# omegaiota/DiffCloth

Hardware: AMD Instinct MI355X
Metric: fwd+bwd steps/sec (node), 10k-vtx cloth+contact, batch=256 (higher is better)
Workload: dtype f32

## Files before the change

diffcloth_amd/capi.py:

```python
import ctypes as C
import os

import numpy as np

_HERE = os.path.dirname(os.path.abspath(__file__))
LIB_PATH = os.path.join(_HERE, "lib", "libdiffcloth_hip.so")

DC_PRIM_SPHERE, DC_PRIM_CAPSULE, DC_PRIM_PLANE, DC_PRIM_BOWL, DC_PRIM_SPHERE_DISCRETIZED = 0, 1, 2, 3, 4


class DcError(RuntimeError):
    pass


class dc_primitive(C.Structure):
    _fields_ = [("kind", C.c_int), ("group", C.c_int), ("center", C.c_double * 3), ("top_offset", C.c_double * 3),
                ("corner2", C.c_double * 3), ("radius", C.c_double), ("length", C.c_double), ("mu", C.c_double), ("rotates", C.c_int)]


class dc_params(C.Structure):
    _fields_ = [("time_step", C.c_double), ("density", C.c_double), ("k_stretch", C.c_double), ("k_bend", C.c_double),
                ("k_att", C.c_double), ("gravity", C.c_double * 3), ("forward_tol", C.c_double),
                ("backward_tol", C.c_double), ("gravity_enabled", C.c_int), ("contact_enabled", C.c_int),
                ("selfcollision_enabled", C.c_int), ("gradient_clipping", C.c_int),
                ("gradient_clipping_threshold", C.c_double), ("pd_iter_cap", C.c_int), ("adjoint_iter_cap", C.c_int),
                ("cg_rel_tol", C.c_double), ("cg_max_iter", C.c_int), ("stall_window", C.c_int),
                ("adjoint_mode", C.c_int), ("adjoint_rel_tol", C.c_double), ("adjoint_block_precond", C.c_int), ("adjoint_fp32_only", C.c_int),
                ("max_self_contacts", C.c_int), ("forward_deflation", C.c_int)]


class dc_step_stats(C.Structure):
    _fields_ = [("converged", C.c_int), ("pd_iters", C.c_int), ("cg_iters", C.c_int), ("prim_contacts", C.c_int),
                ("self_contacts", C.c_int), ("last_xdiff", C.c_float), ("self_overflow", C.c_int)]


class dc_bwd_stats(C.Structure):
    _fields_ = [("converged", C.c_int), ("adjoint_iters", C.c_int), ("cg_iters", C.c_int), ("clipped", C.c_int), ("used_direct", C.c_int),
                ("last_udiff", C.c_float), ("refine_cycles", C.c_int), ("fp64_iters", C.c_int), ("residual_verified", C.c_int), ("workgroups", C.c_int)]


class dc_record(C.Structure):
    _fields_ = [("x", C.POINTER(C.c_double)), ("v", C.POINTER(C.c_double)), ("f", C.POINTER(C.c_double)), ("r", C.POINTER(C.c_double)),
                ("prim", C.POINTER(C.c_int)), ("normal", C.POINTER(C.c_double)), ("x_fixed", C.POINTER(C.c_double)),
                ("self_count", C.POINTER(C.c_int)), ("self_pairs", C.POINTER(C.c_int)), ("self_layer", C.POINTER(C.c_int)),
                ("self_normal", C.POINTER(C.c_double)), ("self_d", C.POINTER(C.c_double))]


EXPORTED_SYMBOLS = [
    "dc_create", "dc_destroy", "dc_last_error", "dc_version", "dc_set_mesh", "dc_set_attachments", "dc_set_params",
    "dc_set_primitives", "dc_build", "dc_default_params", "dc_set_solver", "dc_set_flags", "dc_get_counts", "dc_get_system_matrix",
    "dc_get_vertex_data", "dc_alloc_batch", "dc_set_state", "dc_get_state", "dc_set_mu", "dc_set_uniform_force", "dc_set_vertex_forces", "dc_set_vertex_force_field", "dc_get_force_gradient",
    "dc_step_forward", "dc_get_record", "dc_get_contacts", "dc_get_self_contacts", "dc_step_backward", "dc_rollout_forward",
    "dc_seed_gradient", "dc_rollout_backward", "dc_get_gradient", "dc_get_param_gradients", "dc_get_stats", "dc_sync", "dc_timer_start",
    "dc_timer_stop", "dc_kernel_times", "dc_get_cluster", "dc_set_gradient", "dc_set_fixed_point_schedule", "dc_set_force_schedule",
    "dc_set_seed_schedule", "dc_clear_schedules", "dc_get_states", "dc_get_dxfixed", "dc_get_layout", "dc_get_packet_layout", "dc_comm_unique_id", "dc_comm_init", "dc_allreduce_sum", "dc_comm_destroy",
    "dc_get_deflation", "dc_set_record", "dc_set_trajectory_start", "dc_keep_force_gradients", "dc_get_force_gradients", "dc_use_stream", "dc_set_state_dev", "dc_get_state_dev", "dc_step_forward_dev", "dc_step_backward_dev",
    "dc_get_self_friction_path", "dc_get_adjoint_matrix", "dc_dense_phase_times",
]

_lib = None
_dp = C.POINTER(C.c_double)
_ip = C.POINTER(C.c_int)


def load_library():
    global _lib
    if _lib is None:
        path = os.environ.get("DC_LIB", LIB_PATH)
        if not os.path.exists(path):
            raise DcError(f"{path} not found: run `python -m diffcloth_amd.build` (hipcc, gfx950)")
        lib = C.CDLL(path)
        lib.dc_last_error.restype = C.c_char_p
        lib.dc_version.restype = C.c_char_p
        _lib = lib
    return _lib


def _d(a):
    return a.ctypes.data_as(_dp) if a is not None else None


def _i(a):
    return a.ctypes.data_as(_ip) if a is not None else None


def _f64(a):
    return None if a is None else np.ascontiguousarray(np.asarray(a, dtype=np.float64))


def _i32(a):
    return np.ascontiguousarray(np.asarray(a, dtype=np.int32))


def _stats_to_dict(arr, fields):
    return {f: np.array([getattr(s, f) for s in arr]) for f in fields}


class Engine:

    def __init__(self, device=0):
        self.lib = load_library()
        h = C.c_void_p()
        rc = self.lib.dc_create(C.c_int(device), C.byref(h))
        if rc != 0:
            raise DcError(f"dc_create failed with code {rc}: no HIP device available (there is no CPU fallback)")
        self.h = h
        self.device = device
        self.params = dc_params()
        self.lib.dc_default_params(C.byref(self.params))
        self.N = self.T = self.E = self.Af = 0
        self.B = 0
        self.ngroups = 1

    def close(self):
        if getattr(self, "h", None):
            self.lib.dc_destroy(self.h)
            self.h = None

    def __del__(self):
        try:
            self.close()
        except Exception:
            pass

    def _chk(self, rc):
        if rc != 0:
            raise DcError(f"code {rc}: {self.lib.dc_last_error(self.h).decode()}")

    def set_mesh(self, verts, tris):
        v = _f64(verts).reshape(-1)
        t = _i32(tris).reshape(-1)
        self._chk(self.lib.dc_set_mesh(self.h, C.c_int(v.size // 3), _d(v), C.c_int(t.size // 3), _i(t)))

    def set_attachments(self, vertices):
        a = _i32(vertices).reshape(-1)
        self._chk(self.lib.dc_set_attachments(self.h, C.c_int(a.size), _i(a)))

    def set_params(self, **kw):
        for k, v in kw.items():
            if k == "gravity":
                for d in range(3):
                    self.params.gravity[d] = float(v[d])
            elif hasattr(self.params, k):
                setattr(self.params, k, v)
            else:
                raise KeyError(k)
        self._chk(self.lib.dc_set_params(self.h, C.byref(self.params)))

    def set_solver(self, forward_tol=None, backward_tol=None, gradient_clipping=None, clip_threshold=None, force_direct_adjoint=None):
        p = self.params
        if forward_tol is not None: p.forward_tol = forward_tol
        if backward_tol is not None: p.backward_tol = backward_tol
        if gradient_clipping is not None: p.gradient_clipping = int(gradient_clipping)
        if clip_threshold is not None: p.gradient_clipping_threshold = clip_threshold
        if force_direct_adjoint is not None: p.adjoint_mode = (2 if p.adjoint_mode == 2 else 1) if force_direct_adjoint else 0
        self._chk(self.lib.dc_set_solver(self.h, C.c_double(p.forward_tol), C.c_double(p.backward_tol), C.c_int(p.gradient_clipping),
                                         C.c_double(p.gradient_clipping_threshold), C.c_int(int(p.adjoint_mode in (1, 2)))))

    def set_primitives(self, prims):
        arr = (dc_primitive * max(len(prims), 1))()
        groups = []
        for k, p in enumerate(prims):
            arr[k].kind = p.get("kind", DC_PRIM_SPHERE)
            arr[k].group = p.get("group", k)
            for d in range(3):
                arr[k].center[d] = float(p["center"][d])
                arr[k].top_offset[d] = float(p.get("top_offset", (0, 0, 0))[d])
                arr[k].corner2[d] = float(p.get("corner2", (0, 0, 0))[d])
            arr[k].radius = float(p["radius"])
            arr[k].length = float(p.get("length", 0.0))
            arr[k].mu = float(p.get("mu", 0.0))
            arr[k].rotates = int(p.get("rotates", 0))
            if arr[k].group not in groups:
                groups.append(arr[k].group)
        self.ngroups = max(len(groups), 1)
        self._chk(self.lib.dc_set_primitives(self.h, C.c_int(len(prims)), arr))

    def build(self):
        self._chk(self.lib.dc_build(self.h))
        c = _i32(np.zeros(6))
        self._chk(self.lib.dc_get_counts(self.h, _i(c)))
        self.N, self.T, self.E, self.Af, self.nnz, self.rows = [int(x) for x in c]
        return self

    def system_matrix(self):
        ptr = _i32(np.zeros(self.N + 1)); col = _i32(np.zeros(self.nnz)); val = _f64(np.zeros(self.nnz))
        self._chk(self.lib.dc_get_system_matrix(self.h, _i(ptr), _i(col), _d(val)))
        return ptr, col, val

    def vertex_data(self):
        m = _f64(np.zeros(self.N)); a = _f64(np.zeros(self.N)); r = _f64(np.zeros(self.N))
        self._chk(self.lib.dc_get_vertex_data(self.h, _d(m), _d(a), _d(r)))
        return m, a, r

    def alloc_batch(self, batch, tape_steps):
        self._chk(self.lib.dc_alloc_batch(self.h, C.c_int(batch), C.c_int(tape_steps)))
        self.B = batch
        self.tape = tape_steps

    def _vec(self, a, per):
        a = _f64(a).reshape(-1)
        if a.size != self.B * per:
            raise ValueError(f"expected {self.B}x{per} values, got {a.size}")
        return a

    def set_state(self, slot, x, v):
        x = self._vec(x, 3 * self.N); v = self._vec(v, 3 * self.N)
        self._chk(self.lib.dc_set_state(self.h, C.c_int(slot), _d(x), _d(v)))
# ... 86 lines not shown
        return dict(count=cnt.value, layers=nl.value, pairs=pairs[:n], layer=layer[:n], normal=nrm[:n])

    def step_backward(self, slot, dL_dxnew, dL_dvnew, dL_dxinit=None, dL_dvinit=None, is_start=False):
        n3 = 3 * self.N
        gx = self._vec(dL_dxnew, n3); gv = self._vec(dL_dvnew, n3)
        ix = None if dL_dxinit is None else self._vec(dL_dxinit, n3)
        iv = None if dL_dvinit is None else self._vec(dL_dvinit, n3)
        dx = np.zeros((self.B, n3)); dv = np.zeros((self.B, n3))
        dxf = np.zeros((self.B, max(3 * self.Af, 1))); dmu = np.zeros((self.B, self.ngroups))
        st = (dc_bwd_stats * self.B)()
        self._chk(self.lib.dc_step_backward(self.h, C.c_int(slot), _d(gx), _d(gv), _d(ix), _d(iv), C.c_int(int(is_start)),
                                            _d(dx), _d(dv), _d(dxf), _d(dmu), st))
        out = dict(dL_dx=dx, dL_dv=dv, dL_dxfixed=dxf[:, :3 * self.Af], dL_dmu=dmu)
        out.update(_stats_to_dict(st, ["converged", "adjoint_iters", "cg_iters", "clipped", "used_direct", "last_udiff", "refine_cycles", "fp64_iters", "residual_verified", "workgroups"]))
        return out

    def _tp(self, t, per):
        dev = getattr(self, "device", None)
        import torch
        if t is None:
            return None, 1
        if t.is_cuda and dev is not None and t.device.index != dev:
            raise ValueError(f"tensor on cuda:{t.device.index}, the engine runs on device {dev}")
        if not t.is_cuda or not t.is_contiguous() or t.dtype not in (torch.float32, torch.float64) or t.numel() != per:
            raise ValueError(f"expected a contiguous CUDA float32 / float64 tensor of {per} elements, got {t.dtype} {tuple(t.shape)} on {t.device}")
        return C.c_void_p(t.data_ptr()), int(t.dtype == torch.float32)

    def use_stream(self, stream=None):
        self._chk(self.lib.dc_use_stream(self.h, C.c_void_p(stream.cuda_stream) if stream is not None else None))

    def set_state_dev(self, slot, x, v):
        px, f = self._tp(x, self.B * 3 * self.N); pv, f2 = self._tp(v, self.B * 3 * self.N)
        assert f == f2, "x and v must have one dtype"
        self._chk(self.lib.dc_set_state_dev(self.h, C.c_int(slot), px, pv, C.c_int(f)))

    def get_state_dev(self, slot, x, v):
        px, f = self._tp(x, self.B * 3 * self.N); pv, f2 = self._tp(v, self.B * 3 * self.N)
        assert f == f2, "x and v must have one dtype"
        self._chk(self.lib.dc_get_state_dev(self.h, C.c_int(slot), px, pv, C.c_int(f)))

    def step_forward_dev(self, slot, fixed_pts=None):
        p, f = self._tp(fixed_pts, self.B * 3 * self.Af)
        self._chk(self.lib.dc_step_forward_dev(self.h, C.c_int(slot), p, C.c_int(f)))

    def step_backward_dev(self, slot, gx, gv, dx, dv, dxfixed=None, dmu=None, ix=None, iv=None, is_start=False):
        n = self.B * 3 * self.N
        pgx, f = self._tp(gx, n); pgv, _ = self._tp(gv, n); pdx, f3_ = self._tp(dx, n); pdv, _ = self._tp(dv, n)
        pix, _ = self._tp(ix, n); piv, _ = self._tp(iv, n)
        pxf, _ = self._tp(dxfixed, self.B * 3 * self.Af); pmu, _ = self._tp(dmu, self.B * self.ngroups)
        for t in (gv, dx, dv, ix, iv, dxfixed, dmu):
            assert t is None or t.dtype == gx.dtype, "all tensors of a call must have one dtype"
        self._chk(self.lib.dc_step_backward_dev(self.h, C.c_int(slot), pgx, pgv, pix, piv, C.c_int(int(is_start)), pdx, pdv, pxf, pmu, C.c_int(f)))

    def rollout_forward(self, slot, nsteps):
        self._chk(self.lib.dc_rollout_forward(self.h, C.c_int(slot), C.c_int(nsteps)))

    def seed_gradient(self, slot, target=None, scale=1.0):
        t = None if target is None else _f64(target).reshape(-1)
        self._chk(self.lib.dc_seed_gradient(self.h, C.c_int(slot), _d(t), C.c_double(scale)))

    def set_trajectory_start(self, start_slot):
        self._chk(self.lib.dc_set_trajectory_start(self.h, C.c_int(start_slot)))

    def rollout_backward(self, slot, nsteps):
        self._chk(self.lib.dc_rollout_backward(self.h, C.c_int(slot), C.c_int(nsteps)))

    def set_gradient(self, dL_dx, dL_dv):
        n3 = 3 * self.N
        self._chk(self.lib.dc_set_gradient(self.h, _d(self._vec(dL_dx, n3)), _d(self._vec(dL_dv, n3))))

    def set_fixed_point_schedule(self, slot0, xf):
        xf = np.ascontiguousarray(np.asarray(xf, dtype=np.float64).reshape(-1, self.B, 3 * self.Af))
        self._chk(self.lib.dc_set_fixed_point_schedule(self.h, C.c_int(slot0), C.c_int(xf.shape[0]), _d(xf)))

    def set_force_schedule(self, slot0, nsteps, fu=None, fv_scale=None):
        fu = None if fu is None else np.ascontiguousarray(np.asarray(fu, dtype=np.float64).reshape(nsteps, self.B, 3))
        fs = None if fv_scale is None else np.ascontiguousarray(np.asarray(fv_scale, dtype=np.float64).reshape(nsteps, self.B))
        self._chk(self.lib.dc_set_force_schedule(self.h, C.c_int(slot0), C.c_int(nsteps), _d(fu), _d(fs)))

    def set_seed_schedule(self, slot0, dL_dx, dL_dv=None):
        gx = np.ascontiguousarray(np.asarray(dL_dx, dtype=np.float64).reshape(-1, self.B, 3 * self.N))
        gv = None if dL_dv is None else np.ascontiguousarray(np.asarray(dL_dv, dtype=np.float64).reshape(gx.shape))
        self._chk(self.lib.dc_set_seed_schedule(self.h, C.c_int(slot0), C.c_int(gx.shape[0]), _d(gx), _d(gv)))

    def clear_schedules(self):
        self._chk(self.lib.dc_clear_schedules(self.h))

    def get_states(self, slot0, nslots):
        x = np.zeros((nslots, self.B, 3 * self.N)); v = np.zeros((nslots, self.B, 3 * self.N))
        self._chk(self.lib.dc_get_states(self.h, C.c_int(slot0), C.c_int(nslots), _d(x), _d(v)))
        return x, v

    def get_dxfixed(self, slot0, nslots):
        out = np.zeros((nslots, self.B, max(3 * self.Af, 1)))
        if self.Af > 0:
            out = np.zeros((nslots, self.B, 3 * self.Af))
            self._chk(self.lib.dc_get_dxfixed(self.h, C.c_int(slot0), C.c_int(nslots), _d(out)))
        return out[:, :, :3 * self.Af]

    def get_gradient(self):
        dx = np.zeros((self.B, 3 * self.N)); dv = np.zeros((self.B, 3 * self.N)); dmu = np.zeros((self.B, self.ngroups))
        self._chk(self.lib.dc_get_gradient(self.h, _d(dx), _d(dv), _d(dmu)))
        return dx, dv, dmu

    def get_mu_gradient(self):
        dmu = np.zeros((self.B, self.ngroups))
        self._chk(self.lib.dc_get_gradient(self.h, None, None, _d(dmu)))
        return dmu

    def get_param_gradients(self, slot):
        out = np.zeros((self.B, 8))
        self._chk(self.lib.dc_get_param_gradients(self.h, C.c_int(slot), _d(out)))
        return dict(dL_dk=out[:, 0:3], dL_ddensity=out[:, 3], sum_dfext=out[:, 4:7])

    def get_stats(self, slot):
        f = (dc_step_stats * self.B)(); b = (dc_bwd_stats * self.B)()
        self._chk(self.lib.dc_get_stats(self.h, C.c_int(slot), f, b))
        return (_stats_to_dict(f, ["converged", "pd_iters", "cg_iters", "prim_contacts", "self_contacts", "last_xdiff", "self_overflow"]),
                _stats_to_dict(b, ["converged", "adjoint_iters", "cg_iters", "clipped", "used_direct", "last_udiff", "refine_cycles", "fp64_iters", "residual_verified", "workgroups"]))

    def sync(self):
        self._chk(self.lib.dc_sync(self.h))

    @staticmethod
    def comm_unique_id():
        lib = load_library()
        buf = C.create_string_buffer(128)
        rc = lib.dc_comm_unique_id(buf)
        if rc != 0:
            raise DcError(f"code {rc}: dc_comm_unique_id failed (RCCL not available?)")
        return buf.raw

    def comm_init(self, nranks, rank, unique_id):
        self._chk(self.lib.dc_comm_init(self.h, C.c_int(nranks), C.c_int(rank), C.c_char_p(unique_id)))

    def allreduce_sum(self, values):
        a = np.ascontiguousarray(np.asarray(values, dtype=np.float64).reshape(-1)).copy()
        self._chk(self.lib.dc_allreduce_sum(self.h, _d(a), C.c_int(a.size)))
        return a

    def comm_destroy(self):
        self._chk(self.lib.dc_comm_destroy(self.h))

    def layout(self):
        c = _i32(np.zeros(6))
        self._chk(self.lib.dc_get_layout(self.h, _i(c)))
        return dict(renumbered=bool(c[0]), bandwidth=int(c[1]), packet_kernel=bool(c[2]), element_windows=bool(c[3]), windows=int(c[4]), dense_inverse=bool(c[5]))

    def packet_byte_offsets(self):
        k = C.c_int()
        self._chk(self.lib.dc_get_packet_layout(self.h, C.byref(k)))
        return bool(k.value)

    def deflation(self):
        k = C.c_int(); pi = C.c_int()
        self._chk(self.lib.dc_get_deflation(self.h, C.byref(k), C.byref(pi)))
        return k.value, pi.value

    def cluster(self):
        k = C.c_int(); nb = C.c_int()
        self._chk(self.lib.dc_get_cluster(self.h, C.byref(k), C.byref(nb)))
        return k.value

    def self_friction_path(self, reset=False):
        out = np.zeros((self.B, 2), dtype=np.int32)
        self._chk(self.lib.dc_get_self_friction_path(self.h, _i(out), C.c_int(int(reset))))
        return out

    def timer_start(self):
        self._chk(self.lib.dc_timer_start(self.h))

    def timer_stop(self):
        ms = C.c_float()
        self._chk(self.lib.dc_timer_stop(self.h, C.byref(ms)))
        return ms.value

    def adjoint_matrix(self, slot, rollout):
        n = 3 * self.N
        K = np.zeros((n, n))
        self._chk(self.lib.dc_get_adjoint_matrix(self.h, C.c_int(slot), C.c_int(rollout), _d(K)))
        return K

    def dense_phase_times(self, reset=False):
        ms = (C.c_float * 3)()
        self._chk(self.lib.dc_dense_phase_times(self.h, ms, C.c_int(int(reset))))
        return tuple(float(v) for v in ms)

    def kernel_times(self, reset=False):
        a = C.c_float(); b = C.c_float(); na = C.c_int(); nb = C.c_int()
        self._chk(self.lib.dc_kernel_times(self.h, C.byref(a), C.byref(na), C.byref(b), C.byref(nb), C.c_int(int(reset))))
        return dict(fwd_ms=a.value, fwd_launches=na.value, bwd_ms=b.value, bwd_launches=nb.value)
```

diffcloth_amd/csrc/dc_device.h:

```cpp
#pragma once
#include <hip/hip_runtime.h>
#include "../../include/diffcloth_hip.h"

namespace dc {

constexpr int kMaxPrims = 8;
constexpr int kMaxLayers = 4088;
constexpr int kMetaStride = 4096;

#if defined(__HIP_DEVICE_COMPILE__) && defined(DC_KERNEL_TU)
#define DC_G __attribute__((address_space(1)))
#define DC_C __attribute__((address_space(4)))
#else
#define DC_G
#define DC_C
#endif

struct DevPrim {
  int kind, group, rotates, pad;
  float cx, cy, cz, radius;
  float tx, ty, tz, length;
  float ux, uy, uz, pad2;
};

struct DevSystem {
  int N, T, E, Af, NC;
  int nprim, ngroups, pad0;
  const int DC_G *tri_v;
  const float4 DC_G *tri_D;
  const float DC_G *tri_w2;
  const int DC_G *bend_v;
  const float4 DC_G *bend_w;
  const float2 DC_G *bend_nw;
  const int DC_G *att_vertex;
  const int DC_G *att_of_vertex;
  const float DC_G *mass;
  const float DC_G *dinv;
  const int DC_G *P_ptr;
  const int DC_G *P_col;
  const float DC_G *P_val;
  const int DC_G *inc_ptr;
  const int DC_G *inc_idx;
  const int2 DC_G *ell;
  const int DC_G *ell_ptr;
  const int DC_G *ell_w;
  const int4 DC_G *pk;
  const int DC_C *pk_ptr;
  const int DC_C *pk_n;
  const float DC_G *sq_dinv;
  int pk_vpt, pk_ok;
  int pk_threads;
  int pk_ofs;
  int adj_coarse;
  const double DC_G *dsph_tri;
  int dsph_ntri;
  int fwd_defl;
  const float DC_G *defl_u;
  const float DC_G *defl_au;
  const float DC_C *defl_g;
  const float DC_G *dense_inv;
  int dense_ld;
  const int DC_G *user_of;
  const int DC_G *dev_of;
  const int4 DC_C *win;
  const int4 DC_G *wtri_rec;
  const float4 DC_G *wtri_D;
  const int4 DC_G *wbend_rec;
  const float4 DC_G *wbend_w;
  const float4 DC_G *wtri_Dlo;
  const float4 DC_G *wbend_lo;
  const int4 DC_G *winc;
  const int DC_C *winc_ptr;
  const int DC_C *winc_n;
  int nwin, win_vcap, win_nrcap, win_ok;
  int win_lds_bytes, pad2;
  const float DC_G *radii;
  const int DC_G *conn_ptr;
  const int DC_G *conn_idx;
  float max_radii;
  int self_cap;
  int self_lds;
  float h, k_att, gx, gy, gz;
  float k_stretch, k_bend, density;
  int contact_enabled, self_enabled, pad1;
  const double DC_G *tri_D64;
  const double DC_G *tri_w2_64;
  const double DC_G *bend_w64;
  const double DC_G *bend_nw64;
  const double DC_G *mass64;
  const float4 DC_G *tri_Dlo;
  const float4 DC_G *bend_lo;
  double h64, k_att64, k_stretch64, k_bend64, density64;
  double g64[3];
  DevPrim prims[kMaxPrims];
  const DevSystem *self_dev;
};

struct DevWork {
  float *g;
  float *vnow;
  float *vbest;
  float *cg_r, *cg_p, *cg_ap, *cg_x;
  float *corner;
  float4 *ap4;
  float *pre_p, *pre_s;
  float *minv;
  double *u64, *r64, *y64, *x64, *k64[6];
  double *c64;
  int *sd_cell, *sd_order;
  float *sd_sx;
  int2 *sd_rawpair;
  float4 *sd_rawn;
  int *sd_tmp;
};

struct SelfRec {
  int2 *pair;
  float4 *nrm;
  float4 *dvec;
  int *meta;
  int *verts;
};

struct FwdArgs {
  const float *x_in, *v_in;
  float *x_out, *v_out;
  float *rec_f, *rec_r, *rec_n;
  int *rec_prim;
  const float *x_fixed;
  const float *mu;
  const float *fu;
  const float *fv;
  const float *fv_scale;
  const float *fv2;
  dc_step_stats *stats;
  SelfRec self;
  float fwd_tol, cg_tol;
  int pd_cap, cg_max, stall_window;
  int self_full;
  int cg_seed;
  int nsteps, inline_detect;
  size_t slot_state, slot_prim, slot_stats;
  size_t slot_self, slot_meta;
  size_t slot_xfix, slot_fu, slot_fvs;
};

struct BwdArgs {
  const float *x_new;
  const float *rec_f, *rec_n;
  const int *rec_prim;
  SelfRec self;
  const float *mu;
  float *gx, *gv;
  const float *ix, *iv;
  float *d_xfixed;
  float *d_mu;
  float *d_param;
  const float *x_fixed;
  const float *x_prev, *v_prev;
  const float *v_new;
  dc_bwd_stats *stats;
  float bwd_tol, cg_tol, clip_thr, rel_tol;
  int mode;
  int it_cap, cg_max, is_start, clip, stall_window;
  int block_pre;
  int fp32_only;
  int dense_y;
  int verify_all;
  int cg_first;
  int warm;
  int ycap, ybase;
  int nsteps, slot;
  int start_at;
  size_t slot_state, slot_prim, slot_self, slot_meta, slot_param, slot_xf, slot_stats;
  size_t slot_ix;
  const double *inj_x, *inj_f, *inj_n, *inj_sn, *inj_sd;
  float *ys;
};

void launch_pd_step(const DevSystem &S, const DevWork &W, const FwdArgs &A, int B, hipStream_t st);
bool pd_step_fusable(const DevSystem &S);
bool launch_pd_step_packet(const DevSystem &S, const DevWork &W, const FwdArgs &A, int B, hipStream_t st);
bool launch_pd_step_resident(const DevSystem &S, const DevWork &W, const FwdArgs &A, int B, hipStream_t st, int variant);
void launch_self_detect(const DevSystem &S, const DevWork &W, const FwdArgs &A, int B, hipStream_t st);
void launch_adjoint_step(const DevSystem &S, const DevWork &W, const BwdArgs &A, int B, hipStream_t st);
void launch_f64i_to_f32p(const double *src, float *dst, int B, int n, const int *user_of, hipStream_t st);
void launch_f32p_to_f64i(const float *src, double *dst, int B, int n, const int *user_of, hipStream_t st);
void launch_f64i_to_f64p(const double *src, double *dst, int B, int n, const int *user_of, hipStream_t st);
void launch_dev_to_planar(const void *src, int is_f32, float *dst, int B, int n, const int *user_of, hipStream_t st);
void launch_planar_to_dev(const float *src, void *dst, int is_f32, int B, int n, const int *user_of, hipStream_t st);
void launch_copy_cast(const float *src, void *dst, int is_f32, long total, hipStream_t st);
void launch_seed_gradient(const float *x, const float *target, float *gx, float *gv, int B, int N, float scale, hipStream_t st);

}
```

diffcloth_amd/csrc/dc_engine.hip:

```cpp
#include <hip/hip_runtime.h>
#include <algorithm>
#include <cmath>
#include <cstdio>
#include <cstring>
#include <string>
#include <vector>
#include "dc_clusterplan.h"
#include "dc_context.h"
#include "dc_env.h"
#include "dc_record.h"
#include "dc_tables.h"
#include "dc_spheremesh.h"
#include "dc_selftmp.h"

using namespace dc;

namespace dc {
hipError_t launch_pd_step_cluster(const DevSystem &S, const DevCluster &CL, const DevWork &W, const FwdArgs &A, int b0, int nb, hipStream_t st);
hipError_t launch_adjoint_step_cluster(const DevSystem &S, const DevCluster &CL, const DevWork &W, const BwdArgs &A, int b0, int nb, hipStream_t st);
}

static_assert(rec::kMetaStride == kMetaStride && rec::kMaxLayers == kMaxLayers, "dc_record.h restates dc_device.h's record sizes");
static_assert(sizeof(rec::Int2) == sizeof(int2) && alignof(rec::Int2) == alignof(int2), "dc_record.h: Int2 is uploaded as int2");
static_assert(sizeof(rec::Float4) == sizeof(float4) && alignof(rec::Float4) == alignof(float4), "dc_record.h: Float4 is uploaded as float4");
// ... 76 lines not shown
  if (rc) return rc;
  launch_f32p_to_f64i(src, stage, c->B, n_per_rollout, per_vertex ? c->d_user_of : nullptr, c->stream);
  HIPCHK(c, hipMemcpyAsync(dst, stage, elems * sizeof(double), hipMemcpyDeviceToHost, c->stream));
  return DC_OK;
}

int check_batch(dc_ctx *c, int slot_lo, int slot_hi) {
  if (!c->built) return fail(c, DC_ERR_STATE, "dc_build has not been called");
  if (c->B <= 0) return fail(c, DC_ERR_STATE, "dc_alloc_batch has not been called");
  if (slot_lo < 0 || slot_hi > c->tape) return fail(c, DC_ERR_INVALID, "tape slot out of range");
  return DC_OK;
}

int check_self_overflow(dc_ctx *c, const dc_step_stats *st, int slot) {
  for (int b = 0; b < c->B; b++)
    if (st[b].self_overflow)
      return fail(c, DC_ERR_CAPACITY, "self-contact list overflow in the step that produced slot " + std::to_string(slot) + ", rollout " +
                  std::to_string(b) + ((st[b].self_overflow & 1) ? ": more pairs than max_self_contacts = " + std::to_string(c->self_cap) : (st[b].self_overflow & 2) ? std::string(": more than 4088 contact layers") : std::string(": inconsistent contact tables (internal error)")) +
                  " (raise dc_params::max_self_contacts and repeat the step)");
  return DC_OK;
}

FwdArgs fwd_args(dc_ctx *c, int slot) {
  const size_t se = slot_elems(c), sp = (size_t) c->B * c->host.N;
  FwdArgs A;
  A.x_in = c->X + se * slot; A.v_in = c->V + se * slot;
  A.x_out = c->X + se * (slot + 1); A.v_out = c->V + se * (slot + 1);
  A.rec_f = c->F + se * (slot + 1); A.rec_r = c->R + se * (slot + 1); A.rec_n = c->NRM + se * (slot + 1);
  A.rec_prim = c->PRIM + sp * (slot + 1);
  A.x_fixed = c->xf_cur; A.mu = c->mu; A.fu = c->fu_set ? c->fu : nullptr; A.fv = c->fv_set ? c->fv : nullptr;
  A.fv2 = c->fv2_set ? c->fv2 : nullptr;
  A.fv_scale = nullptr; A.slot_xfix = 0; A.slot_fu = 0; A.slot_fvs = 0;
  if (c->S.Af > 0 && c->sched_xf[slot + 1]) A.x_fixed = xf_slot(c, slot + 1);
  if (c->sched_fu[slot + 1]) A.fu = c->FU_S + (size_t) c->B * 3 * (slot + 1);
  if (c->sched_fvs[slot + 1] && A.fv) A.fv_scale = c->FVS_S + (size_t) c->B * (slot + 1);
  A.stats = c->fstats + (size_t) c->B * (slot + 1);
  A.self = self_slot(c, slot + 1);
  A.fwd_tol = (float) c->params.forward_tol;
  A.cg_tol = (float) (c->params.cg_rel_tol > 0 ? c->params.cg_rel_tol : 1e-4);
  A.pd_cap = pd_cap(c);
  A.cg_max = c->params.cg_max_iter > 0 ? c->params.cg_max_iter : 500;
  A.stall_window = c->params.stall_window > 0 ? c->params.stall_window : 0x7fffffff;
  static const bool seed_on = env_not_off("DC_CG_SEED", true);
  A.cg_seed = seed_on ? 1 : 0;
  A.self_full = env_on("DC_FWD_SELFFULL", false);
  A.nsteps = 1; A.inline_detect = 0; A.slot_state = se; A.slot_prim = sp; A.slot_stats = (size_t) c->B;
  A.slot_self = (size_t) c->B * c->self_cap; A.slot_meta = (size_t) c->B * kMetaStride;
  return A;
}
enum class Seeds { none, init, schedule };
BwdArgs bwd_args(dc_ctx *c, int slot, bool is_start, Seeds seeds) {
  const size_t se = slot_elems(c), sp = (size_t) c->B * c->host.N;
  BwdArgs A;
  A.x_new = c->X + se * slot; A.rec_f = c->F + se * slot; A.rec_n = c->NRM + se * slot;
  A.rec_prim = c->PRIM + sp * slot; A.mu = c->mu;
  A.self = self_slot(c, slot);
  A.gx = c->GX; A.gv = c->GV;
  A.ix = nullptr; A.iv = nullptr; A.slot_ix = 0;
  if (seeds == Seeds::init) { A.ix = c->IX; A.iv = c->IV; }
  if (seeds == Seeds::schedule && c->SEEDX && c->sched_seed[slot - 1]) { A.ix = seedx_slot(c, slot - 1); A.iv = seedv_slot(c, slot - 1); A.slot_ix = se; }
  A.d_xfixed = dxf_slot(c, slot); A.d_mu = c->DMU;
  A.d_param = dpar_slot(c, slot);
  A.x_fixed = xf_slot(c, slot);
  A.x_prev = c->X + se * (slot - 1); A.v_prev = c->V + se * (slot - 1); A.v_new = c->V + se * slot; A.stats = c->bstats + (size_t) c->B * slot;
  A.bwd_tol = (float) c->params.backward_tol;
  A.cg_tol = (float) (c->params.cg_rel_tol > 0 ? c->params.cg_rel_tol : 1e-4);
  A.clip_thr = (float) c->params.gradient_clipping_threshold;
  A.it_cap = c->params.adjoint_iter_cap > 0 ? c->params.adjoint_iter_cap : 400;
  A.cg_max = c->params.cg_max_iter > 0 ? c->params.cg_max_iter : 500;
  A.is_start = is_start; A.clip = c->params.gradient_clipping;
  A.start_at = c->start_slot + 1;
  A.mode = c->params.adjoint_mode;
  A.rel_tol = (float) (c->params.adjoint_rel_tol > 0 ? c->params.adjoint_rel_tol : 1e-6);
  A.stall_window = c->params.stall_window > 0 ? c->params.stall_window : 0x7fffffff;
  A.block_pre = env_not_off("DC_BLOCK_PRE", c->params.adjoint_block_precond != 0);
  A.fp32_only = env_on("DC_ADJ_FP32", c->params.adjoint_fp32_only != 0);
  A.dense_y = env_on("DC_ADJ_DENSEY", false);
  A.verify_all = env_on("DC_ADJ_VERIFY", false);
  A.warm = env_on("DC_ADJ_WARM", false);
  A.cg_first = env_on("DC_ADJ_CG", true);
  A.ycap = 0; A.ybase = 0;
  A.nsteps = 1; A.slot = slot;
  const bool inj = c->inj_slot == slot && c->INJ_X;
  A.inj_x = inj ? c->INJ_X : nullptr; A.inj_f = inj ? c->INJ_F : nullptr; A.inj_n = inj ? c->INJ_N : nullptr;
  A.inj_sn = inj ? c->INJ_SN : nullptr; A.inj_sd = inj ? c->INJ_SD : nullptr;
  A.ys = (c->keep_y && c->YS) ? c->YS + se * slot : nullptr;
  A.slot_state = se; A.slot_prim = sp; A.slot_self = (size_t) c->B * c->self_cap; A.slot_meta = (size_t) c->B * kMetaStride;
  A.slot_param = (size_t) c->B * 8; A.slot_xf = xf_elems(c); A.slot_stats = (size_t) c->B;
  return A;
}


void free_cluster(dc_ctx *c) {
  for (void *p : c->cl.allocs) (void) hipFree(p);
  c->cl = ClusterSet();
}

int upload_cluster(dc_ctx *c, const ClusterPlan &P) {
  ClusterSet &cl = c->cl;
  DevCluster &D = cl.D;
  std::memset(&D, 0, sizeof(D));
  D.K = P.K; D.R = P.R; D.HB = P.HB; D.wpp = P.wpp; D.nb = P.nb; D.xch_stride = P.xch_stride; D.pk_vpt = P.pk_vpt;
  D.spin_limit = P.spin_limit; D.redundant_self = P.redundant_self; D.test_drop = P.test_drop; D.test_skew = P.test_skew;
  const HostWindows &HW = P.win;
  const HostPackets &HP = P.pk;
  D.nwin = HW.nwin; D.win_vcap = HW.vcap; D.win_nrcap = HW.nrcap; D.win_lds_bytes = (int) HW.lds_bytes;
  const struct { const void *src; size_t count; void *dst; } tables[] = {
    {HW.win.data(), HW.win.size(), &D.win}, {HW.tri_rec.data(), HW.tri_rec.size(), &D.wtri_rec}, {HW.tri_D.data(), HW.tri_D.size(), &D.wtri_D},
    {HW.bend_rec.data(), HW.bend_rec.size(), &D.wbend_rec}, {HW.bend_w.data(), HW.bend_w.size(), &D.wbend_w},
    {HW.tri_Dlo.data(), HW.tri_Dlo.size(), &D.wtri_Dlo}, {HW.bend_lo.data(), HW.bend_lo.size(), &D.wbend_lo},
    {HW.inc.data(), HW.inc.size(), &D.winc}, {HW.inc_ptr.data(), HW.inc_ptr.size(), &D.winc_ptr}, {HW.inc_n.data(), HW.inc_n.size(), &D.winc_n},
    {HP.pk.data(), HP.pk.size(), &D.pk}, {HP.pk_ptr.data(), HP.pk_ptr.size(), &D.pk_ptr}, {HP.pk_n.data(), HP.pk_n.size(), &D.pk_n},
    {HP.sq_dinv.data(), HP.sq_dinv.size(), &D.sq_dinv}};
  static_assert(sizeof(int) == 4 && sizeof(float) == 4, "4-byte table elements");
  int rc;
  for (const auto &t : tables) {
    int *p = nullptr;
    if ((rc = dev_alloc(c, cl.allocs, &p, t.count))) return rc;
    if (t.count) HIPCHK(c, hipMemcpy(p, t.src, t.count * 4, hipMemcpyHostToDevice));
    std::memcpy(t.dst, &p, sizeof(p));
  }
  if ((rc = dev_alloc(c, cl.allocs, &D.xch, P.xch_bytes / sizeof(v4i)))) return rc;
  if ((rc = dev_alloc(c, cl.allocs, &D.err, 4))) return rc;
  if ((rc = dev_alloc(c, cl.allocs, &D.self_path, 2 * (size_t) c->B))) return rc;
  DevCluster *dD = nullptr;
  if ((rc = dev_alloc(c, cl.allocs, &dD, 1))) return rc;
  D.self_dev = dD;
  HIPCHK(c, hipMemcpy(dD, &D, sizeof(DevCluster), hipMemcpyHostToDevice));
  cl.K = P.K; cl.nb = P.nb; cl.xch_bytes = P.xch_bytes;
  cl.ok = true;
  return DC_OK;
}

static int deflation_want(const dc_params &p) {
  if (env_set("DC_DEFLATION")) return env_int("DC_DEFLATION", 0) > 0 ? 16 : 0;
  return p.forward_deflation > 0 ? 16 : p.forward_deflation;
}
static bool build_deflation_cached(dc_ctx *c, const HostSystem &H, int want, int rows_padded, HostDeflation **out) {
  uint64_t h = 1469598103934665603ull;
  auto mix = [&](const void *q, size_t n) { const unsigned char *b = (const unsigned char *) q; for (size_t i = 0; i < n; i++) { h ^= b[i]; h *= 1099511628211ull; } };
  mix(&H.N, sizeof(int)); mix(&want, sizeof(int)); mix(&rows_padded, sizeof(int));
  mix(H.P_ptr.data(), H.P_ptr.size() * sizeof(H.P_ptr[0])); mix(H.P_col.data(), H.P_col.size() * sizeof(H.P_col[0]));
  mix(H.P_val.data(), H.P_val.size() * sizeof(H.P_val[0])); mix(H.mass.data(), H.mass.size() * sizeof(H.mass[0]));
  if (!c->defl_cache_valid || c->defl_key != h) {
    c->defl_cache_built = c->defl_cache.build(H, want, rows_padded);
    c->defl_key = h; c->defl_cache_valid = true;
  }
  *out = &c->defl_cache;
  return c->defl_cache_built;
}

static void set_decisions(DevSystem &S, const HostTables &plan) {
  S.win_ok = plan.win_ok; S.nwin = plan.nwin; S.pk_ok = plan.pk_ok; S.pk_vpt = plan.pk_vpt; S.pk_threads = plan.pk_threads;
  S.pk_ofs = plan.pk_ofs;
  S.fwd_defl = plan.fwd_defl; S.adj_coarse = plan.adj_coarse; S.dense_ld = plan.dense_ld;
  S.max_radii = plan.max_radii; S.self_cap = plan.self_cap; S.self_lds = plan.self_lds;
}

int choose_cluster(dc_ctx *c) {
  free_cluster(c);
  ClusterSwitches sw;
  sw.forced = env_int("DC_CLUSTER", -1);
  sw.redundant_self = env_on("DC_SELF_REDUNDANT", true);
  sw.spin_ms = env_int("DC_TEST_SPIN_MS", 0);
  sw.test_drop = env_on("DC_TEST_DROP_PART", false);
  sw.test_skew = env_int("DC_TEST_SKEW_PART", -1);
  ClusterPlan plan;
  plan.build(c->host, c->bandwidth, c->B, c->cus, c->host_only, c->S.pk_ok != 0, c->S.win_ok != 0, c->S.dense_inv != nullptr, sw);
  return plan.ok ? upload_cluster(c, plan) : DC_OK;
}

int cluster_check(dc_ctx *c) {
  if (!c->cl.ok) return DC_OK;
  unsigned e[4] = {0, 0, 0, 0};
  HIPCHK(c, hipMemcpy(e, c->cl.D.err, sizeof(e), hipMemcpyDeviceToHost));
  if (e[0]) HIPCHK(c, hipMemset(c->cl.D.err, 0, 16));
  if (e[0]) return fail(c, DC_ERR_HIP, "split kernels: an inter-workgroup exchange timed out (waiting for sequence " + std::to_string(e[1]) + ", saw tag " +
                        std::to_string(e[2]) + ", site " + std::to_string(e[3] & 255u) + ", part " + std::to_string((e[3] >> 8) & 15u) + ", granule " +
                        std::to_string(e[3] >> 12) + "; set DC_CLUSTER=1 to run one workgroup per rollout)");
  return DC_OK;
}

bool use_cluster_fwd(const dc_ctx *c) { return c->cl.ok; }
bool use_cluster_bwd(const dc_ctx *c) { return c->cl.ok && c->params.adjoint_mode == 1; }

int check_dense_mode(dc_ctx *c, int mode, int N, const char *who) {
  if (mode == 2 && N > kDenseMaxN)
    return fail(c, DC_ERR_INVALID, std::string(who) + ": adjoint_mode 2 (dense direct adjoint solve) is limited to meshes of at most " +
                std::to_string(kDenseMaxN) + " vertices; this mesh has " + std::to_string(N));
  return DC_OK;
}

int dense_ensure(dc_ctx *c) {
  if (c->dense.K) return DC_OK;
  const int N = c->host.N, ld = dense_adj_ld(N), cap = std::max(c->self_cap, 1);
  const size_t per = (size_t) ld * ld * sizeof(double) + (size_t) ld * sizeof(int) + sizeof(int) + (size_t) 9 * N * sizeof(double) +
                     (size_t) 9 * cap * sizeof(double);
  const size_t budget = (size_t) 8 << 30;
  int nb = (int) std::max<size_t>(1, std::min<size_t>((size_t) c->B, budget / per));
  const int chunk = env_int("DC_DENSE_CHUNK", 0);
  if (chunk > 0) nb = std::min(nb, chunk);
  int rc;
  DenseAdjWork &D = c->dense;
  D.ld = ld;
  if ((rc = dev_alloc(c, c->batch_allocs, &D.K, (size_t) nb * ld * ld))) return rc;
  if ((rc = dev_alloc(c, c->batch_allocs, &D.piv, (size_t) nb * ld))) return rc;
  if ((rc = dev_alloc(c, c->batch_allocs, &D.flag, (size_t) nb))) return rc;
  if ((rc = dev_alloc(c, c->batch_allocs, &D.pm, (size_t) nb * 9 * N))) return rc;
  if ((rc = dev_alloc(c, c->batch_allocs, &D.sg, (size_t) nb * 9 * cap))) return rc;
  c->dense_nb = nb;
  c->dense_timing = env_on("DC_DENSE_TIMES", false);
  if (c->dense_timing)
    for (auto &e : c->ev_d) if (!e) HIPCHK(c, hipEventCreate(&e));
  return DC_OK;
}

int enqueue_dense_adjoint(dc_ctx *c, const BwdArgs &A) {
  if (A.nsteps != 1) return fail(c, DC_ERR_INVALID, "adjoint_mode 2 runs one backward step per launch");
  int rc;
  if ((rc = dense_ensure(c))) return rc;
  const DenseAdjWork &D = c->dense;
  const int n = 3 * c->host.N;
  static const int one = 1;
  const int forced = env_int("DC_DENSE_FLAG", -1);
  for (int b0 = 0; b0 < c->B; b0 += c->dense_nb) {
    const int nb = std::min(c->dense_nb, c->B - b0);
    if (c->dense_timing) HIPCHK(c, hipEventRecord(c->ev_d[0], c->stream));
    HIPCHK(c, hipMemsetAsync(D.flag, 0, sizeof(int) * nb, c->stream));
    if (forced >= b0 && forced < b0 + nb) HIPCHK(c, hipMemcpyAsync(D.flag + (forced - b0), &one, sizeof(int), hipMemcpyHostToDevice, c->stream));
    launch_dense_assemble(c->S, A, c->W.x64, D, b0, nb, c->stream);
    if (c->dense_timing) HIPCHK(c, hipEventRecord(c->ev_d[1], c->stream));
    c->dense_launches += 2 + launch_dense_factor(D, n, nb, c->stream);
    if (c->dense_timing) HIPCHK(c, hipEventRecord(c->ev_d[2], c->stream));
    launch_dense_adjoint_step(c->S, c->W, A, D, b0, nb, c->stream);
    c->dense_launches += 1;
    HIPCHK(c, hipGetLastError());
    if (c->dense_timing) {
      HIPCHK(c, hipEventRecord(c->ev_d[3], c->stream));
      HIPCHK(c, hipEventSynchronize(c->ev_d[3]));
      for (int k = 0; k < 3; k++) {
        float ms = 0;
        HIPCHK(c, hipEventElapsedTime(&ms, c->ev_d[k], c->ev_d[k + 1]));
        c->dense_ms[k] += ms;
      }
    }
  }
  return DC_OK;
}

int enqueue_pd_step(dc_ctx *c, const FwdArgs &A) {
  {
    const long first = (long) ((A.x_out - c->X) / (long) slot_elems(c));
    if (c->inj_slot >= first && c->inj_slot < first + A.nsteps) c->inj_slot = -1;
  }
  if (!use_cluster_fwd(c)) { launch_pd_step(c->S, c->W, A, c->B, c->stream); HIPCHK(c, hipGetLastError()); return DC_OK; }
  for (int b0 = 0; b0 < c->B; b0 += c->cl.nb) {
    HIPCHK(c, hipMemsetAsync(c->cl.D.xch, 0, c->cl.xch_bytes, c->stream));
    HIPCHK(c, launch_pd_step_cluster(c->S, c->cl.D, c->W, A, b0, std::min(c->cl.nb, c->B - b0), c->stream));
  }
  return DC_OK;
}
int enqueue_adjoint_step(dc_ctx *c, const BwdArgs &A) {
  if (c->params.adjoint_mode == 2) return enqueue_dense_adjoint(c, A);
  if (!use_cluster_bwd(c)) { launch_adjoint_step(c->S, c->W, A, c->B, c->stream); HIPCHK(c, hipGetLastError()); return DC_OK; }
  for (int b0 = 0; b0 < c->B; b0 += c->cl.nb) {
    HIPCHK(c, hipMemsetAsync(c->cl.D.xch, 0, c->cl.xch_bytes, c->stream));
    HIPCHK(c, launch_adjoint_step_cluster(c->S, c->cl.D, c->W, A, b0, std::min(c->cl.nb, c->B - b0), c->stream));
  }
  return DC_OK;
}

bool fuse_steps_enabled() {
  static const bool on = env_not_off("DC_FUSE_STEPS", true);
  return on;
}

int enqueue_forward_steps(dc_ctx *c, int slot, int nsteps, bool carry_targets, int *launches) {
  const bool self_on = c->S.contact_enabled && c->S.self_enabled, has_xf = c->S.Af > 0;
  const bool fused = fuse_steps_enabled() && nsteps > 1 && (use_cluster_fwd(c) || pd_step_fusable(c->S));
  const size_t xf_bytes = sizeof(float) * xf_elems(c);
  int rc;
  FwdArgs FA = fwd_args(c, slot);
  if (fused) {
    int nxf = 0, nfu = 0, nfvs = 0;
    for (int k = 1; k <= nsteps; k++) { nxf += c->sched_xf[slot + k]; nfu += c->sched_fu[slot + k]; nfvs += c->sched_fvs[slot + k]; }
    if ((nxf % nsteps) || (nfu % nsteps) || (nfvs % nsteps))
      return fail(c, DC_ERR_INVALID, "dc_rollout_forward: a fixed-point / force schedule covers only part of the steps " + std::to_string(slot) + " .. " + std::to_string(slot + nsteps));
    if (nxf) FA.slot_xfix = xf_elems(c);
    if (nfu) FA.slot_fu = (size_t) c->B * 3;
    if (nfvs && FA.fv_scale) FA.slot_fvs = (size_t) c->B;
    FA.nsteps = nsteps; FA.inline_detect = self_on ? 1 : 0;
  }
  for (int k = 0; k < nsteps; k++) {
    if (has_xf && !c->sched_xf[slot + k + 1]) HIPCHK(c, hipMemcpyAsync(xf_slot(c, slot + k + 1), c->xf_cur, xf_bytes, hipMemcpyDeviceToDevice, c->stream));
    if (fused) continue;
    if (k) FA = fwd_args(c, slot + k);
    if (self_on) launch_self_detect(c->S, c->W, FA, c->B, c->stream);
    if ((rc = enqueue_pd_step(c, FA))) return rc;
  }
  if (fused && (rc = enqueue_pd_step(c, FA))) return rc;
  if (carry_targets && has_xf && c->sched_xf[slot + nsteps])
    HIPCHK(c, hipMemcpyAsync(c->xf_cur, xf_slot(c, slot + nsteps), xf_bytes, hipMemcpyDeviceToDevice, c->stream));
  if (launches) *launches = fused ? 1 : nsteps;
  return DC_OK;
}

int enqueue_backward_steps(dc_ctx *c, int slot, int nsteps, Seeds seeds, const bool *is_start, int *launches) {
// ... 42 lines not shown

extern "C" {

const char *dc_version(void) { return "diffcloth_hip 0.1 (gfx950)"; }

void dc_default_params(dc_params *p) {
  std::memset(p, 0, sizeof(*p));
  p->time_step = 1.0 / 90; p->density = 0.1; p->k_stretch = 100; p->k_bend = 0.01; p->k_att = 10000;
  p->gravity[0] = 0; p->gravity[1] = -9.8; p->gravity[2] = 0;
  p->forward_tol = 1e-7; p->backward_tol = 5e-5;
  p->gravity_enabled = 1; p->contact_enabled = 1; p->selfcollision_enabled = 0;
  p->gradient_clipping = 1; p->gradient_clipping_threshold = 16.0;
  p->pd_iter_cap = -1; p->adjoint_iter_cap = 400; p->cg_rel_tol = 1e-4; p->cg_max_iter = 500; p->stall_window = 0;
  p->adjoint_mode = 0; p->adjoint_rel_tol = 1e-6; p->adjoint_block_precond = 1; p->adjoint_fp32_only = 0;
  p->max_self_contacts = 0;
  p->forward_deflation = -1;
}

int dc_create(int device_id, dc_ctx **out) {
  if (!out) return DC_ERR_INVALID;
  *out = nullptr;
  if (device_id == -1) {
    dc_ctx *c = new dc_ctx();
    c->device = -1; c->host_only = true;
    dc_default_params(&c->params);
    std::memset(&c->S, 0, sizeof(c->S));
    std::memset(&c->W, 0, sizeof(c->W));
    *out = c;
    return DC_OK;
  }
  int count = 0;
  if (hipGetDeviceCount(&count) != hipSuccess || count <= 0) return DC_ERR_HIP;
  if (device_id < 0 || device_id >= count) return DC_ERR_INVALID;
  dc_ctx *c = new dc_ctx();
  c->device = device_id;
  dc_default_params(&c->params);
  std::memset(&c->S, 0, sizeof(c->S));
  std::memset(&c->W, 0, sizeof(c->W));
  if (hipSetDevice(device_id) != hipSuccess || hipStreamCreate(&c->stream) != hipSuccess) { delete c; return DC_ERR_HIP; }
  c->own_stream = c->stream;
  if (hipDeviceGetAttribute(&c->cus, hipDeviceAttributeMultiprocessorCount, device_id) != hipSuccess || c->cus <= 0) c->cus = 256;
  if (hipEventCreate(&c->ev_a) != hipSuccess || hipEventCreate(&c->ev_b) != hipSuccess || hipEventCreate(&c->ev_t0) != hipSuccess ||
      hipEventCreate(&c->ev_t1) != hipSuccess) { delete c; return DC_ERR_HIP; }
  *out = c;
  return DC_OK;
}

int dc_destroy(dc_ctx *c) {
  if (!c) return DC_OK;
  if (c->host_only) { delete c; return DC_OK; }
  (void) hipSetDevice(c->device);
  (void) hipStreamSynchronize(c->stream);
  (void) dc_comm_destroy(c);
  free_cluster(c);
  free_pool(c->table_allocs);
  free_pool(c->batch_allocs);
  (void) hipEventDestroy(c->ev_a); (void) hipEventDestroy(c->ev_b);
  (void) hipEventDestroy(c->ev_t0); (void) hipEventDestroy(c->ev_t1);
  for (hipEvent_t e : c->ev_d) if (e) (void) hipEventDestroy(e);
  (void) hipStreamDestroy(c->own_stream);
  delete c;
  return DC_OK;
}

const char *dc_last_error(const dc_ctx *c) { return c ? c->err.c_str() : "null context"; }

int dc_set_mesh(dc_ctx *c, int n, const double *pos, int t, const int *tris) {
  if (!c) return DC_ERR_INVALID;
  c->built = false;
  c->user_of.clear(); c->dev_of.clear();
  if (!c->host.set_mesh(n, pos, t, tris)) { c->mesh_set = false; return fail(c, DC_ERR_TOPOLOGY, c->host.error); }
  const bool env = env_set("DC_RENUMBER");
  const bool want = env_on("DC_RENUMBER", 2 * mesh_bandwidth(t, tris) > 511);
  if (want) {
    std::vector<int> order = rcm_order(n, t, tris);
    std::vector<int> inv(n);
    for (int k = 0; k < n; k++) inv[order[k]] = k;
    std::vector<int> tri2(3 * (size_t) t);
    for (size_t k = 0; k < tri2.size(); k++) tri2[k] = inv[tris[k]];
    if (2 * mesh_bandwidth(t, tri2.data()) < 2 * mesh_bandwidth(t, tris) || env) {
      std::vector<double> pos2(3 * (size_t) n);
      for (int k = 0; k < n; k++) for (int d = 0; d < 3; d++) pos2[3 * (size_t) k + d] = pos[3 * (size_t) order[k] + d];
      if (!c->host.set_mesh(n, pos2.data(), t, tri2.data())) { c->mesh_set = false; return fail(c, DC_ERR_TOPOLOGY, c->host.error); }
      c->user_of = order; c->dev_of = inv;
    }
  }
  c->mesh_set = true;
  return DC_OK;
}

int dc_set_attachments(dc_ctx *c, int count, const int *vertex) {
  if (!c || count < 0 || (count > 0 && !vertex)) return fail(c, DC_ERR_INVALID, "dc_set_attachments: bad arguments");
  c->att_user.assign(vertex, vertex + count);
  c->built = false;
  return DC_OK;
}

int dc_set_params(dc_ctx *c, const dc_params *p) {
  if (!c || !p) return DC_ERR_INVALID;
  if (!(p->time_step > 0) || !(p->density > 0)) return fail(c, DC_ERR_INVALID, "dc_set_params: time_step and density must be > 0");
  if (c->mesh_set) { const int rc = check_dense_mode(c, p->adjoint_mode, c->host.N, "dc_set_params"); if (rc) return rc; }
  c->params = *p;
  c->built = false;
  return DC_OK;
}

int dc_set_primitives(dc_ctx *c, int count, const dc_primitive *prims) {
  if (!c || count < 0 || count > kMaxPrims) return fail(c, DC_ERR_INVALID, "dc_set_primitives: at most 8 flattened primitives");
  if (count > 0 && !prims) return fail(c, DC_ERR_INVALID, "dc_set_primitives: null primitive array");
  int discretised = 0;
  for (int k = 0; k < count; k++) {
    if (prims[k].kind < DC_PRIM_SPHERE || prims[k].kind > DC_PRIM_SPHERE_DISCRETIZED) return fail(c, DC_ERR_INVALID, "dc_set_primitives: unknown primitive kind");
    if (prims[k].kind == DC_PRIM_SPHERE_DISCRETIZED) {
      discretised++;
      if (!(prims[k].radius > 0) || prims[k].length < 0 || prims[k].length > 512) return fail(c, DC_ERR_INVALID, "dc_set_primitives: discretised sphere needs radius > 0 and a resolution (length) of 0 or 3 ... 512");
    }
  }
  if (discretised > 1) return fail(c, DC_ERR_INVALID, "dc_set_primitives: at most one discretised sphere per context");
  c->prims.assign(prims, prims + count);
  std::vector<int> seen;
  c->group_of_prim.assign(count, 0);
  for (int k = 0; k < count; k++) {
    int g = -1;
    for (size_t s = 0; s < seen.size(); s++) if (seen[s] == prims[k].group) g = (int) s;
    if (g < 0) { g = (int) seen.size(); seen.push_back(prims[k].group); }
    c->group_of_prim[k] = g;
  }
  c->ngroups = (int) seen.size();
  c->built = false;
  return DC_OK;
}

int dc_build(dc_ctx *c) {
  if (!c) return DC_ERR_INVALID;
  if (!c->mesh_set) return fail(c, DC_ERR_STATE, "dc_build: dc_set_mesh has not been called");
  { const int rc = check_dense_mode(c, c->params.adjoint_mode, c->host.N, "dc_build"); if (rc) return rc; }
  c->inj_slot = -1;
  const dc_params &p = c->params;
  HostSystem &H = c->host;
  H.att_vertex = c->att_user;
  for (int &a : H.att_vertex) {
    if (a < 0 || a >= H.N) return fail(c, DC_ERR_INVALID, "dc_build: attachment vertex out of range");
    if (!c->dev_of.empty()) a = c->dev_of[a];
  }
  if (!H.build_numerics(p.time_step, p.density, p.k_stretch, p.k_bend, p.k_att)) return fail(c, DC_ERR_TOPOLOGY, H.error);
  TableSwitches sw;
  sw.windows = env_not_off("DC_WINDOWS", true);
  sw.dense_max_n = env_int("DC_DENSE_MAX_N", kDenseMaxN);
  sw.self_lds = env_not_off("DC_SELF_LDS", true);
  static const bool adj_coarse = env_int("DC_ADJ_COARSE", 1) != 0;
  sw.adj_coarse = adj_coarse;
  sw.pk_h16 = pk_h16_enabled() != 0;
  sw.pk_ofs = env_not_off("DC_PK_OFS", true);
  HostTables plan;
  plan.build(H, p, sw);
  HostDeflation *HD = nullptr;
  const bool defl = plan.defl_rows > 0 && build_deflation_cached(c, H, deflation_want(p), plan.defl_rows, &HD);
  plan.set_deflation(defl, sw);
  c->bandwidth = plan.bandwidth;
  c->defl_k = HD ? HD->k : 0; c->defl_probe = HD ? HD->probe_iterations : 0;
  DevSystem &S = c->S;
  if (c->host_only) {
    std::memset(&S, 0, sizeof(S));
    set_decisions(S, plan);
    c->built = true;
    return DC_OK;
  }
  HIPCHK(c, hipSetDevice(c->device));
  HIPCHK(c, hipStreamSynchronize(c->stream));
  free_cluster(c);
  free_pool(c->table_allocs);
  std::memset(&S, 0, sizeof(S));
  set_decisions(S, plan);
  S.N = H.N; S.T = H.T; S.E = H.E; S.Af = (int) H.att_vertex.size(); S.NC = 3 * H.T + 4 * H.E;
  c->d_user_of = nullptr;
  int rc;
  if (!c->user_of.empty()) {
    if ((rc = upload<int>(c, &S.user_of, c->user_of))) return rc;
    if ((rc = upload<int>(c, &S.dev_of, c->dev_of))) return rc;
    c->d_user_of = S.user_of;
  }
  if ((rc = upload<int>(c, &S.tri_v, plan.tri_v))) return rc;
  if ((rc = upload_as<float>(c, &S.tri_D, H.tri_D))) return rc;
  if ((rc = upload<float>(c, &S.tri_w2, H.tri_w2))) return rc;
  if ((rc = upload<int>(c, &S.bend_v, plan.bend_v))) return rc;
  if ((rc = upload_as<float>(c, &S.bend_w, H.bend_w))) return rc;
  if ((rc = upload_as<float>(c, &S.bend_nw, plan.bend_nw))) return rc;
  if ((rc = upload<int>(c, &S.att_vertex, H.att_vertex))) return rc;
  if ((rc = upload<int>(c, &S.att_of_vertex, plan.att_of_vertex))) return rc;
  if ((rc = upload<float>(c, &S.mass, H.mass))) return rc;
  if ((rc = upload<float>(c, &S.dinv, plan.dinv))) return rc;
  if ((rc = upload<double>(c, &S.tri_D64, plan.tri_D64))) return rc;
  if ((rc = upload<double>(c, &S.tri_w2_64, H.tri_w2))) return rc;
  if ((rc = upload<double>(c, &S.bend_w64, plan.bend_w64))) return rc;
  if ((rc = upload<double>(c, &S.bend_nw64, plan.bend_nw64))) return rc;
  if ((rc = upload<double>(c, &S.mass64, H.mass))) return rc;
  if ((rc = upload_as<float>(c, &S.tri_Dlo, plan.tri_Dlo))) return rc;
  if ((rc = upload_as<float>(c, &S.bend_lo, plan.bend_lo))) return rc;
  if ((rc = upload<int>(c, &S.P_ptr, H.P_ptr))) return rc;
  if ((rc = upload<int>(c, &S.P_col, H.P_col))) return rc;
  if ((rc = upload<float>(c, &S.P_val, H.P_val))) return rc;
  if ((rc = upload<int>(c, &S.inc_ptr, H.inc_ptr))) return rc;
  if ((rc = upload<int>(c, &S.inc_idx, H.inc_idx))) return rc;
  if ((rc = upload<float>(c, &S.radii, H.radii))) return rc;
  if ((rc = upload<int>(c, &S.conn_ptr, H.conn_ptr))) return rc;
  if ((rc = upload<int>(c, &S.conn_idx, H.conn_idx))) return rc;
  if ((rc = upload_as<int>(c, &S.ell, plan.ell))) return rc;
  if ((rc = upload<int>(c, &S.ell_ptr, plan.ell_ptr))) return rc;
  if ((rc = upload<int>(c, &S.ell_w, plan.ell_w))) return rc;
  if (plan.win_ok) {
    const HostWindows &HW = plan.win;
    if ((rc = upload_as<int>(c, &S.win, HW.win))) return rc;
    if ((rc = upload_as<int>(c, &S.wtri_rec, HW.tri_rec))) return rc;
    if ((rc = upload_as<float>(c, &S.wtri_D, HW.tri_D))) return rc;
    if ((rc = upload_as<int>(c, &S.wbend_rec, HW.bend_rec))) return rc;
    if ((rc = upload_as<float>(c, &S.wbend_w, HW.bend_w))) return rc;
    if ((rc = upload_as<float>(c, &S.wtri_Dlo, HW.tri_Dlo))) return rc;
    if ((rc = upload_as<float>(c, &S.wbend_lo, HW.bend_lo))) return rc;
    if ((rc = upload_as<int>(c, &S.winc, HW.inc))) return rc;
    if ((rc = upload<int>(c, &S.winc_ptr, HW.inc_ptr))) return rc;
    if ((rc = upload<int>(c, &S.winc_n, HW.inc_n))) return rc;
    S.win_vcap = HW.vcap; S.win_nrcap = HW.nrcap; S.win_lds_bytes = (int) HW.lds_bytes;
  }
  if (plan.pk_ok) {
    if ((rc = upload_as<int>(c, &S.pk, plan.pk.pk))) return rc;
    if ((rc = upload<int>(c, &S.pk_ptr, plan.pk.pk_ptr))) return rc;
    if ((rc = upload<int>(c, &S.pk_n, plan.pk.pk_n))) return rc;
  }
  if ((rc = upload<float>(c, &S.sq_dinv, plan.pk_ok ? plan.pk.sq_dinv : plan.sq_dinv))) return rc;
  if (defl) {
    if ((rc = upload<float>(c, &S.defl_u, HD->U))) return rc;
    if ((rc = upload<float>(c, &S.defl_au, HD->AU))) return rc;
    if ((rc = upload<float>(c, &S.defl_g, HD->G))) return rc;
  }
  if (plan.dense_ld && (rc = upload<float>(c, &S.dense_inv, plan.dense.inv))) return rc;
  S.h = (float) p.time_step; S.k_att = (float) p.k_att;
  S.k_stretch = (float) p.k_stretch; S.k_bend = (float) p.k_bend; S.density = (float) p.density;
  S.gx = p.gravity_enabled ? (float) p.gravity[0] : 0.f;
  S.gy = p.gravity_enabled ? (float) p.gravity[1] : 0.f;
  S.gz = p.gravity_enabled ? (float) p.gravity[2] : 0.f;
  S.h64 = p.time_step; S.k_att64 = p.k_att; S.k_stretch64 = p.k_stretch; S.k_bend64 = p.k_bend; S.density64 = p.density;
  for (int k = 0; k < 3; k++) S.g64[k] = p.gravity_enabled ? p.gravity[k] : 0.0;
  S.contact_enabled = p.contact_enabled; S.self_enabled = p.selfcollision_enabled;
  S.nprim = (int) c->prims.size(); S.ngroups = std::max(c->ngroups, 1);
  S.dsph_tri = nullptr; S.dsph_ntri = 0;
  for (int k = 0; k < S.nprim; k++) {
    const dc_primitive &q = c->prims[k];
    if (q.kind == DC_PRIM_SPHERE_DISCRETIZED) {
      const int res = q.length >= 3 ? (int) q.length : 40;
      const std::vector<double> tab = sphere_mesh_table(q.radius, res);
      if ((rc = upload<double>(c, &S.dsph_tri, tab))) return rc;
      S.dsph_ntri = (int) tab.size() / 12;
    }
    DevPrim &d = S.prims[k];
    d.kind = q.kind; d.group = c->group_of_prim[k]; d.rotates = q.rotates; d.pad = 0;
    d.cx = (float) q.center[0]; d.cy = (float) q.center[1]; d.cz = (float) q.center[2]; d.radius = (float) q.radius;
    d.tx = (float) q.top_offset[0]; d.ty = (float) q.top_offset[1]; d.tz = (float) q.top_offset[2]; d.length = (float) q.length;
    d.ux = (float) q.corner2[0]; d.uy = (float) q.corner2[1]; d.uz = (float) q.corner2[2]; d.pad2 = 0.f;
  }
  {
    DevSystem *dS = nullptr;
    if ((rc = dev_alloc(c, c->table_allocs, &dS, 1))) return rc;
    S.self_dev = dS;
    HIPCHK(c, hipMemcpy(dS, &S, sizeof(DevSystem), hipMemcpyHostToDevice));
  }
  c->built = true;
  if (c->B > 0) {
    int B = c->B, tape = c->tape;
    c->B = 0;
    return dc_alloc_batch(c, B, tape);
  }
  return DC_OK;
}

int dc_set_solver(dc_ctx *c, double forward_tol, double backward_tol, int gradient_clipping, double clip_threshold, int force_direct_adjoint) {
  if (!c) return DC_ERR_INVALID;
  c->params.forward_tol = forward_tol; c->params.backward_tol = backward_tol;
  c->params.gradient_clipping = gradient_clipping; c->params.gradient_clipping_threshold = clip_threshold;
  c->params.adjoint_mode = force_direct_adjoint ? (c->params.adjoint_mode == 2 ? 2 : 1) : 0;
  return DC_OK;
}

int dc_set_flags(dc_ctx *c, int gravity_enabled, int contact_enabled, int selfcollision_enabled) {
  if (!c) return DC_ERR_INVALID;
  c->params.gravity_enabled = gravity_enabled; c->params.contact_enabled = contact_enabled;
  c->params.selfcollision_enabled = selfcollision_enabled;
  if (!c->built || c->host_only) return DC_OK;
  DevSystem &S = c->S;
  S.gx = gravity_enabled ? (float) c->params.gravity[0] : 0.f;
  S.gy = gravity_enabled ? (float) c->params.gravity[1] : 0.f;
  S.gz = gravity_enabled ? (float) c->params.gravity[2] : 0.f;
  for (int k = 0; k < 3; k++) S.g64[k] = gravity_enabled ? c->params.gravity[k] : 0.0;
  S.contact_enabled = contact_enabled; S.self_enabled = selfcollision_enabled;
  HIPCHK(c, hipStreamSynchronize(c->stream));
  HIPCHK(c, hipMemcpy((void *) S.self_dev, &S, sizeof(DevSystem), hipMemcpyHostToDevice));
  return DC_OK;
}

int dc_get_counts(const dc_ctx *c, int *out6) {
  if (!c || !out6 || !c->mesh_set) return DC_ERR_INVALID;
  out6[0] = c->host.N; out6[1] = c->host.T; out6[2] = c->host.E; out6[3] = (int) c->host.att_vertex.size();
  out6[4] = (int) c->host.P_col.size(); out6[5] = c->host.rows();
  return DC_OK;
}
int dc_get_system_matrix(const dc_ctx *c, int *row_ptr, int *col, double *val) {
  if (!c || !c->built) return DC_ERR_STATE;
  const HostSystem &H = c->host;
  if (c->user_of.empty()) {
    std::memcpy(row_ptr, H.P_ptr.data(), sizeof(int) * H.P_ptr.size());
    std::memcpy(col, H.P_col.data(), sizeof(int) * H.P_col.size());
    std::memcpy(val, H.P_val.data(), sizeof(double) * H.P_val.size());
    return DC_OK;
  }
  row_ptr[0] = 0;
  std::vector<std::pair<int, double>> row;
  for (int u = 0; u < H.N; u++) {
    const int i = c->dev_of[u];
    row.clear();
    for (int k = H.P_ptr[i]; k < H.P_ptr[i + 1]; k++) row.push_back({c->user_of[H.P_col[k]], H.P_val[k]});
    std::sort(row.begin(), row.end());
    for (size_t k = 0; k < row.size(); k++) { col[row_ptr[u] + k] = row[k].first; val[row_ptr[u] + k] = row[k].second; }
    row_ptr[u + 1] = row_ptr[u] + (int) row.size();
  }
  return DC_OK;
}
int dc_get_vertex_data(const dc_ctx *c, double *mass, double *area, double *radii) {
  if (!c || !c->built) return DC_ERR_STATE;
  const int N = c->host.N;
  for (int i = 0; i < N; i++) {
    const int u = c->user_of.empty() ? i : c->user_of[i];
    if (mass) mass[u] = c->host.mass[i];
    if (area) area[u] = c->host.area[i];
    if (radii) radii[u] = c->host.radii[i];
  }
  return DC_OK;
}

int dc_alloc_batch(dc_ctx *c, int B, int tape) {
  if (!c) return DC_ERR_INVALID;
  if (c->host_only) return fail(c, DC_ERR_STATE, "host-only context (dc_create(-1)): no device, and there is no CPU compute path");
  if (!c->built) return fail(c, DC_ERR_STATE, "dc_alloc_batch: dc_build has not been called");
  if (B <= 0 || tape <= 0) return fail(c, DC_ERR_INVALID, "dc_alloc_batch: batch and tape_steps must be > 0");
  HIPCHK(c, hipSetDevice(c->device));
  HIPCHK(c, hipStreamSynchronize(c->stream));
  free_pool(c->batch_allocs);
  c->dense = DenseAdjWork{}; c->dense_nb = 0;
  c->B = B; c->tape = tape; c->start_slot = 0;
  const int N = c->host.N, Af = (int) c->host.att_vertex.size(), NC = c->S.NC, G = c->S.ngroups;
  const size_t se = (size_t) B * 3 * N, slots = (size_t) tape + 1;
  auto &pool = c->batch_allocs;
  int rc;
  if ((rc = dev_alloc(c, pool, &c->X, se * slots))) return rc;
  if ((rc = dev_alloc(c, pool, &c->V, se * slots))) return rc;
  if ((rc = dev_alloc(c, pool, &c->F, se * slots))) return rc;
  if ((rc = dev_alloc(c, pool, &c->R, se * slots))) return rc;
  if ((rc = dev_alloc(c, pool, &c->NRM, se * slots))) return rc;
  if ((rc = dev_alloc(c, pool, &c->PRIM, (size_t) B * N * slots))) return rc;
  if ((rc = dev_alloc(c, pool, &c->W.g, se))) return rc;
  if ((rc = dev_alloc(c, pool, &c->W.vnow, se))) return rc;
  if ((rc = dev_alloc(c, pool, &c->W.vbest, se))) return rc;
  if ((rc = dev_alloc(c, pool, &c->W.cg_r, se))) return rc;
  if ((rc = dev_alloc(c, pool, &c->W.cg_p, se))) return rc;
  if ((rc = dev_alloc(c, pool, &c->W.cg_ap, se))) return rc;
  if ((rc = dev_alloc(c, pool, &c->W.cg_x, se))) return rc;
  if ((rc = dev_alloc(c, pool, &c->W.corner, (size_t) B * 3 * NC))) return rc;
  if ((rc = dev_alloc(c, pool, &c->W.ap4, (size_t) B * N))) return rc;
  if ((rc = dev_alloc(c, pool, &c->W.pre_p, se))) return rc;
  if ((rc = dev_alloc(c, pool, &c->W.pre_s, se))) return rc;
  if ((rc = dev_alloc(c, pool, &c->W.minv, (size_t) B * 9 * N))) return rc;
  if ((rc = dev_alloc(c, pool, &c->W.u64, se))) return rc;
  if ((rc = dev_alloc(c, pool, &c->W.r64, se))) return rc;
  if ((rc = dev_alloc(c, pool, &c->W.y64, se))) return rc;
  if ((rc = dev_alloc(c, pool, &c->W.x64, se))) return rc;
  if ((rc = dev_alloc(c, pool, &c->W.c64, (size_t) B * 3 * NC))) return rc;
// ... 438 lines not shown
  if (dL_dv && (rc = d2h_planar(c, c->GV, dL_dv, N, true))) return rc;
  if ((rc = stage_sync(c))) return rc;
  if (dL_dmu) {
    std::vector<float> dmu((size_t) c->B * G);
    HIPCHK(c, hipMemcpy(dmu.data(), c->DMU, dmu.size() * sizeof(float), hipMemcpyDeviceToHost));
    for (size_t k = 0; k < dmu.size(); k++) dL_dmu[k] = dmu[k];
  }
  return DC_OK;
}

int dc_set_fixed_point_schedule(dc_ctx *c, int slot0, int nsteps, const double *xf) {
  int rc = check_batch(c, slot0, slot0 + nsteps);
  if (rc) return rc;
  if (nsteps < 1 || !xf) return fail(c, DC_ERR_INVALID, "dc_set_fixed_point_schedule: null schedule");
  const int Af = c->S.Af;
  if (Af <= 0) return DC_OK;
  HIPCHK(c, hipSetDevice(c->device));
  const size_t per = xf_elems(c);
  for (int k = 0; k < nsteps; k++) {
    if ((rc = h2d_planar(c, xf + per * k, xf_slot(c, slot0 + k + 1), Af, false))) return rc;
    c->sched_xf[slot0 + k + 1] = 1;
  }
  return stage_sync(c);
}

int dc_set_force_schedule(dc_ctx *c, int slot0, int nsteps, const double *fu, const double *fv_scale) {
  int rc = check_batch(c, slot0, slot0 + nsteps);
  if (rc) return rc;
  if (nsteps < 1) return fail(c, DC_ERR_INVALID, "dc_set_force_schedule: nsteps < 1");
  HIPCHK(c, hipSetDevice(c->device));
  HIPCHK(c, hipStreamSynchronize(c->stream));
  if (fu) {
    std::vector<float> v((size_t) nsteps * c->B * 3);
    for (size_t k = 0; k < v.size(); k++) v[k] = (float) fu[k];
    HIPCHK(c, hipMemcpy(c->FU_S + (size_t) c->B * 3 * (slot0 + 1), v.data(), v.size() * sizeof(float), hipMemcpyHostToDevice));
  }
  if (fv_scale) {
    std::vector<float> v((size_t) nsteps * c->B);
    for (size_t k = 0; k < v.size(); k++) v[k] = (float) fv_scale[k];
    HIPCHK(c, hipMemcpy(c->FVS_S + (size_t) c->B * (slot0 + 1), v.data(), v.size() * sizeof(float), hipMemcpyHostToDevice));
  }
  for (int k = 1; k <= nsteps; k++) { c->sched_fu[slot0 + k] = fu ? 1 : 0; c->sched_fvs[slot0 + k] = fv_scale ? 1 : 0; }
  return DC_OK;
}

int dc_set_seed_schedule(dc_ctx *c, int slot0, int nslots, const double *dL_dx, const double *dL_dv) {
  int rc = check_batch(c, slot0, slot0 + nslots - 1);
  if (rc) return rc;
  if (nslots < 1 || !dL_dx) return fail(c, DC_ERR_INVALID, "dc_set_seed_schedule: null schedule");
  HIPCHK(c, hipSetDevice(c->device));
  const size_t se = slot_elems(c), slots = (size_t) c->tape + 1;
  if (!c->SEEDX) {
    if ((rc = dev_alloc(c, c->batch_allocs, &c->SEEDX, se * slots))) return rc;
    if ((rc = dev_alloc(c, c->batch_allocs, &c->SEEDV, se * slots))) return rc;
  }
  const int N = c->host.N;
  for (int k = 0; k < nslots; k++) {
    if ((rc = h2d_planar(c, dL_dx + se * k, seedx_slot(c, slot0 + k), N, true))) return rc;
    if (dL_dv) { if ((rc = h2d_planar(c, dL_dv + se * k, seedv_slot(c, slot0 + k), N, true))) return rc; }
    else HIPCHK(c, hipMemsetAsync(seedv_slot(c, slot0 + k), 0, se * sizeof(float), c->stream));
    c->sched_seed[slot0 + k] = 1;
  }
  return stage_sync(c);
}

int dc_clear_schedules(dc_ctx *c) {
  if (!c || c->B <= 0) return fail(c, DC_ERR_STATE, "dc_clear_schedules: no batch");
  std::fill(c->sched_xf.begin(), c->sched_xf.end(), 0); std::fill(c->sched_fu.begin(), c->sched_fu.end(), 0);
  std::fill(c->sched_fvs.begin(), c->sched_fvs.end(), 0); std::fill(c->sched_seed.begin(), c->sched_seed.end(), 0);
  return DC_OK;
}

int dc_set_gradient(dc_ctx *c, const double *dL_dx, const double *dL_dv) {
  int rc = check_batch(c, 0, 0);
  if (rc) return rc;
  if (!dL_dx || !dL_dv) return fail(c, DC_ERR_INVALID, "dc_set_gradient: null gradient");
  HIPCHK(c, hipSetDevice(c->device));
  if ((rc = h2d_planar(c, dL_dx, c->GX, c->host.N, true))) return rc;
  if ((rc = h2d_planar(c, dL_dv, c->GV, c->host.N, true))) return rc;
  HIPCHK(c, hipMemsetAsync(c->DMU, 0, sizeof(float) * c->B * c->S.ngroups, c->stream));
  return stage_sync(c);
}

int dc_get_states(dc_ctx *c, int slot0, int nslots, double *x, double *v) {
  int rc = check_batch(c, slot0, slot0 + nslots - 1);
  if (rc) return rc;
  if (nslots < 1) return fail(c, DC_ERR_INVALID, "dc_get_states: nslots < 1");
  HIPCHK(c, hipSetDevice(c->device));
  const size_t se = slot_elems(c);
  for (int k = 0; k < nslots; k++) {
    if (x && (rc = d2h_planar(c, c->X + se * (slot0 + k), x + se * k, c->host.N, true))) return rc;
    if (v && (rc = d2h_planar(c, c->V + se * (slot0 + k), v + se * k, c->host.N, true))) return rc;
  }
  return stage_sync(c);
}

int dc_get_dxfixed(dc_ctx *c, int slot0, int nslots, double *dL_dxfixed) {
  int rc = check_batch(c, slot0, slot0 + nslots - 1);
  if (rc) return rc;
  if (slot0 < 1 || nslots < 1 || !dL_dxfixed) return fail(c, DC_ERR_INVALID, "dc_get_dxfixed: slot 0 has no record");
  const int Af = c->S.Af;
  if (Af <= 0) return DC_OK;
  HIPCHK(c, hipSetDevice(c->device));
  const size_t per = xf_elems(c);
  for (int k = 0; k < nslots; k++)
    if ((rc = d2h_planar(c, dxf_slot(c, slot0 + k), dL_dxfixed + per * k, Af, false))) return rc;
  return stage_sync(c);
}

int dc_get_param_gradients(dc_ctx *c, int slot, double *out) {
  int rc = check_batch(c, slot, slot);
  if (rc) return rc;
  if (slot < 1 || !out) return fail(c, DC_ERR_INVALID, "dc_get_param_gradients: slot 0 has no record");
  HIPCHK(c, hipSetDevice(c->device));
  HIPCHK(c, hipStreamSynchronize(c->stream));
  std::vector<float> v((size_t) c->B * 8);
  HIPCHK(c, hipMemcpy(v.data(), dpar_slot(c, slot), v.size() * sizeof(float), hipMemcpyDeviceToHost));
  for (size_t k = 0; k < v.size(); k++) out[k] = v[k];
  return DC_OK;
}

int dc_get_stats(dc_ctx *c, int slot, dc_step_stats *fwd, dc_bwd_stats *bwd) {
  int rc = check_batch(c, slot, slot);
  if (rc) return rc;
  HIPCHK(c, hipStreamSynchronize(c->stream));
  if (fwd) HIPCHK(c, hipMemcpy(fwd, c->fstats + (size_t) c->B * slot, sizeof(dc_step_stats) * c->B, hipMemcpyDeviceToHost));
  if (fwd && slot >= 1 && (rc = check_self_overflow(c, fwd, slot))) return rc;
  if (bwd) HIPCHK(c, hipMemcpy(bwd, c->bstats + (size_t) c->B * slot, sizeof(dc_bwd_stats) * c->B, hipMemcpyDeviceToHost));
  return DC_OK;
}

int dc_sync(dc_ctx *c) {
  if (!c) return DC_ERR_INVALID;
  if (c->host_only) return DC_OK;
  HIPCHK(c, hipStreamSynchronize(c->stream));
  return cluster_check(c);
}

int dc_get_deflation(const dc_ctx *c, int *vectors, int *probe_iterations) {
  if (!c) return DC_ERR_INVALID;
  if (!c->built) return DC_ERR_STATE;
  if (vectors) *vectors = c->defl_k;
  if (probe_iterations) *probe_iterations = c->defl_probe;
  return DC_OK;
}

int dc_get_packet_layout(const dc_ctx *c, int *byte_offsets) {
  if (!c || !byte_offsets) return DC_ERR_INVALID;
  if (!c->built) return DC_ERR_STATE;
  *byte_offsets = c->S.pk_ofs;
  return DC_OK;
}

int dc_get_layout(const dc_ctx *c, int *out6) {
  if (!c || !out6) return DC_ERR_INVALID;
  if (!c->built) return DC_ERR_STATE;
  out6[0] = c->user_of.empty() ? 0 : 1; out6[1] = c->bandwidth; out6[2] = c->S.pk_ok; out6[3] = c->S.win_ok; out6[4] = c->S.nwin;
  out6[5] = c->S.dense_ld > 0 ? 1 : 0;
  return DC_OK;
}

int dc_get_cluster(const dc_ctx *c, int *workgroups_per_rollout, int *rollouts_per_launch) {
  if (!c) return DC_ERR_INVALID;
  if (workgroups_per_rollout) *workgroups_per_rollout = c->cl.ok ? c->cl.K : 1;
  if (rollouts_per_launch) *rollouts_per_launch = c->cl.ok ? c->cl.nb : c->B;
  return DC_OK;
}

int dc_get_self_friction_path(dc_ctx *c, int *out, int reset) {
  if (!c || !out) return DC_ERR_INVALID;
  std::memset(out, 0, sizeof(int) * 2 * (size_t) std::max(c->B, 0));
  if (!c->cl.ok || c->B <= 0) return DC_OK;
  HIPCHK(c, hipStreamSynchronize(c->stream));
  HIPCHK(c, hipMemcpy(out, c->cl.D.self_path, sizeof(int) * 2 * (size_t) c->B, hipMemcpyDeviceToHost));
  if (reset) HIPCHK(c, hipMemsetAsync(c->cl.D.self_path, 0, sizeof(int) * 2 * (size_t) c->B, c->stream));
  return DC_OK;
}

int dc_timer_start(dc_ctx *c) {
  if (!c) return DC_ERR_INVALID;
  HIPCHK(c, hipEventRecord(c->ev_t0, c->stream));
  return DC_OK;
}
int dc_timer_stop(dc_ctx *c, float *ms) {
  if (!c || !ms) return DC_ERR_INVALID;
  HIPCHK(c, hipEventRecord(c->ev_t1, c->stream));
  HIPCHK(c, hipEventSynchronize(c->ev_t1));
  HIPCHK(c, hipEventElapsedTime(ms, c->ev_t0, c->ev_t1));
  return DC_OK;
}
int dc_get_adjoint_matrix(dc_ctx *c, int slot, int rollout, double *K) {
  int rc = check_batch(c, slot, slot);
  if (rc) return rc;
  if (slot < 1 || rollout < 0 || rollout >= c->B || !K) return fail(c, DC_ERR_INVALID, "dc_get_adjoint_matrix: bad slot / rollout / output");
  const int N = c->host.N, n = 3 * N;
  if ((rc = check_dense_mode(c, 2, N, "dc_get_adjoint_matrix"))) return rc;
  HIPCHK(c, hipSetDevice(c->device));
  if ((rc = dense_ensure(c))) return rc;
  const DenseAdjWork &D = c->dense;
  launch_dense_assemble(c->S, bwd_args(c, slot, false, Seeds::none), c->W.x64, D, rollout, 1, c->stream);
  HIPCHK(c, hipGetLastError());
  std::vector<double> Kd((size_t) D.ld * n);
  HIPCHK(c, hipMemcpyAsync(Kd.data(), D.K, Kd.size() * sizeof(double), hipMemcpyDeviceToHost, c->stream));
  HIPCHK(c, hipStreamSynchronize(c->stream));
  for (int cj = 0; cj < 3; cj++)
    for (int j = 0; j < N; j++) {
      const int uj = c->user_of.empty() ? j : c->user_of[j];
      const double *col = Kd.data() + (size_t) (cj * N + j) * D.ld;
      for (int ci = 0; ci < 3; ci++)
        for (int i = 0; i < N; i++) {
          const int ui = c->user_of.empty() ? i : c->user_of[i];
          K[(size_t) (3 * ui + ci) * n + 3 * uj + cj] = col[ci * N + i];
        }
    }
  return DC_OK;
}

int dc_dense_phase_times(dc_ctx *c, float *ms3, int reset) {
  if (!c || !ms3) return DC_ERR_INVALID;
  for (int k = 0; k < 3; k++) ms3[k] = c->dense_ms[k];
  if (reset) for (float &v : c->dense_ms) v = 0;
  return DC_OK;
}

int dc_kernel_times(dc_ctx *c, float *fwd_ms, int *fwd_launches, float *bwd_ms, int *bwd_launches, int reset) {
  if (!c) return DC_ERR_INVALID;
  if (fwd_ms) *fwd_ms = c->fwd_ms;
  if (fwd_launches) *fwd_launches = c->fwd_launches;
  if (bwd_ms) *bwd_ms = c->bwd_ms;
  if (bwd_launches) *bwd_launches = c->bwd_launches;
  if (reset) { c->fwd_ms = c->bwd_ms = 0; c->fwd_launches = c->bwd_launches = 0; }
  return DC_OK;
}

}
```

diffcloth_amd/csrc/dc_forward_pk_kernel.h:

```cpp
#pragma once
#include "dc_devlib.h"
#include "dc_winlib.h"
#include "dc_denselib.h"
#include "dc_selflib.h"
#include "dc_pklib.h"
#include "dc_launch.h"
#include <algorithm>


namespace dc {

#ifdef DC_PROFILE_PHASES
#define PH_DECL long long ph_t = clock64(); long long ph_acc[6] = {0, 0, 0, 0, 0, 0}; if (blockIdx.x == 0 && threadIdx.x == 0) { g_win_ph[0] = g_win_ph[1] = g_win_ph[2] = g_win_ph[3] = 0; }
#define PH(k) { long long n_ = clock64(); ph_acc[k] += n_ - ph_t; ph_t = n_; }
#define PH_PRINT if (blockIdx.x == 0 && threadIdx.x == 0) printf("[phases pk] pd %d cg %d | per PD iter: local %lld vertex %lld pd-update %lld | per CG iter: spmv %lld pAp-red %lld upd+red %lld cycles | windows per PD iter: stage %lld tri %lld bend %lld vertex %lld\n", iters, cg_total, ph_acc[0] / iters, ph_acc[1] / iters, ph_acc[5] / iters, ph_acc[2] / max(cg_total, 1), ph_acc[3] / max(cg_total, 1), ph_acc[4] / max(cg_total, 1), g_win_ph[0] / iters, g_win_ph[1] / iters, g_win_ph[2] / iters, g_win_ph[3] / iters);
#else
#define PH_DECL
#define PH(k)
#define PH_PRINT
#endif

template <int THREADS, int VPT, int XL, bool DETECT, bool DENSE, bool H16, bool DEFL, bool OFS>
__device__ __forceinline__ void pd_step_pk(const DevSystem *__restrict__ Sp, const DevWork &W, const FwdArgs &A) {
  static_assert(!(H16 && DENSE), "the explicit-inverse solve keeps the fp32 planes");
  static_assert(H16 || !OFS, "byte offsets address the direction's 8-byte rows");
  const DevSystem &S = *Sp;
  constexpr int NP = THREADS * VPT;
  constexpr int WAVES = THREADS / 64;
  constexpr int XR = VPT - XL;
  constexpr int PF = H16 ? 2 : 3;
  extern __shared__ float lp[];
  float *lx = lp + PF * NP;
  h4 *lh = (h4 *) lp;
  const unsigned lh_addr = lds_byte_address(lp);
  float *ldense = lp + 3 * THREADS * (VPT + XL);
  __shared__ double red[THREADS / 64];
  __shared__ double red2[H16 ? 2 * (THREADS / 64) : 1];
  const int b = blockIdx.x, tid = threadIdx.x, lane = tid & 63;
  const int wv = __builtin_amdgcn_readfirstlane(tid >> 6);
  const int N = S.N, T = S.T, E = S.E, NC = S.NC;
  const size_t off = (size_t) b * 3 * N;
  float *g = W.g + off, *vnow = W.vnow + off, *vbest = W.vbest + off;
  float *dprev = W.cg_x + off;
  float *corner = W.corner + (size_t) b * 3 * NC;
  unsigned tbl_lo = 0, tbl_hi = 0;
  int tbl_n = 0;
  if constexpr (H16) {
    const int ch = wv + min(lane, VPT - 1) * WAVES;
    const unsigned long long a = (unsigned long long) (S.pk + S.pk_ptr[ch]);
    tbl_lo = (unsigned) a; tbl_hi = (unsigned) (a >> 32); tbl_n = S.pk_n[ch];
  }
  for (int step = 0; step < A.nsteps; step++) {
  if (step > 0) __syncthreads();
  const size_t so = (size_t) step * A.slot_state;
  const float *xn = A.x_in + off + so, *vn = A.v_in + off + so;
  float *rec_f = A.rec_f + off + so, *rec_r = A.rec_r + off + so, *rec_n = A.rec_n + off + so;
  int *rec_prim = A.rec_prim + (size_t) b * N + (size_t) step * A.slot_prim;
  const float *xfix = A.x_fixed + (size_t) step * A.slot_xfix + (size_t) b * 3 * S.Af;
  const float *fu_s = A.fu ? A.fu + (size_t) step * A.slot_fu : nullptr;
  const float *fvs_s = A.fv_scale ? A.fv_scale + (size_t) step * A.slot_fvs : nullptr;
  SelfRec srec = A.self;
  srec.pair += (size_t) step * A.slot_self; srec.nrm += (size_t) step * A.slot_self; srec.dvec += (size_t) step * A.slot_self;
  srec.meta += (size_t) step * A.slot_meta; srec.verts += (size_t) step * 2 * A.slot_self;
  if constexpr (DETECT) {
    self_detect_rollout<THREADS>(S, W, b, A.x_in + so, A.v_in + so, A.rec_prim + (size_t) step * A.slot_prim, srec, fu_s, A.fv, fvs_s, (int *) lp, A.fv2);
    __syncthreads();
  }
  const float *mu = A.mu + (size_t) b * S.ngroups;
  const float h = S.h;
  const f3 grav = mk(S.gx, S.gy, S.gz);
  const f3 fu = fu_s ? mk(fu_s[3 * b], fu_s[3 * b + 1], fu_s[3 * b + 2]) : mk(0, 0, 0);
  const float fvs = fvs_s ? fvs_s[b] : 1.f;

  float part = 0.f;
  int ncontact = 0;
  for (int i = tid; i < N; i += THREADS) {
    const float m = S.mass[i];
    f3 v = ld3(vn, i, N);
    f3 fext = grav * m + fu;
    if (A.fv) fext = fext + ld3(A.fv + off, i, N) * fvs;
    if (A.fv2) fext = fext + ld3(A.fv2 + off, i, N);
    f3 v0 = v + fext * (h / m);
    st3(vnow, i, N, v0);
    st3(g, i, N, v0 * m);
    part += dot(v0, v0);
    int prim = -1;
    f3 nrm = mk(0, 0, 0);
    if (S.contact_enabled) prim = detect_primitive(S, ld3(xn, i, N), v0, nrm);
    rec_prim[i] = prim;
    st3(rec_n, i, N, nrm);
    ncontact += (prim >= 0);
  }
  double min_xdiff = (double) h * sqrt(block_sum<THREADS>((double) part, red)) / (double) N;
  const int total_contacts = (int) block_sum<THREADS>((double) ncontact, red);
  const int nself = (S.contact_enabled && S.self_enabled) ? srec.meta[(size_t) b * kMetaStride] : 0;
  bool improved = false, converged = false, stalled = false, best_is_current = false;
  int iters = 0, cg_total = 0, since_progress = 0;
  double xdiff = 0;
  float dnorm = 0.f;

  PH_DECL
  for (int iter = 0; iter < A.pd_cap; iter++) {
    int zp;
    asm volatile("s_mov_b32 %0, 0" : "=s"(zp));
    const int tq = tid + zp;
    auto vertex_body = [&](int i, f3 fint) -> f3 {
      f3 f = ld3(g, i, N) + fint;
      f3 v = ld3(vnow, i, N);
      const int a = S.att_of_vertex[i];
      if (a >= 0) f = f + ((ld3(xfix, a, S.Af) - ld3(xn, i, N)) - v * h) * (h * S.k_att);
      const float m = S.mass[i];
      f3 r = mk(0, 0, 0);
      const int prim = rec_prim[i];
      if (prim >= 0) {
        f3 n = ld3(rec_n, i, N);
        f3 d = f - prim_vout(S.prims[prim], n) * m;
        r = dry_friction(n, d, mu[S.prims[prim].group]);
      }
      st3(rec_f, i, N, f);
      st3(rec_r, i, N, r);
      return (f + r - v * m) * S.sq_dinv[i];
    };
    part = 0.f;
    bool self_done = false;
    if (S.win_ok) {
      float *scr = W.cg_r + off;
#ifndef DC_FWD_NO_VPRE
      struct VIn { f3 g, v; int a; float m; int prim; float sq; };
      auto vert = vert_with_pre_noa([&](int i) {
        VIn q;
        q.g = ld3(g, i, N); q.v = ld3(vnow, i, N); q.a = S.att_of_vertex[i]; q.m = S.mass[i]; q.prim = rec_prim[i]; q.sq = S.sq_dinv[i];
        return q;
      }, [&](int i, f3 fint, f3, const VIn &q) {
        f3 f = q.g + fint;
        if (q.a >= 0) f = f + ((ld3(xfix, q.a, S.Af) - ld3(xn, i, N)) - q.v * h) * (h * S.k_att);
        f3 r = mk(0, 0, 0);
        if (q.prim >= 0) {
          f3 n = ld3(rec_n, i, N);
          f3 d = f - prim_vout(S.prims[q.prim], n) * q.m;
          r = dry_friction(n, d, mu[S.prims[q.prim].group]);
        }
        st3(rec_f, i, N, f);
        st3(rec_r, i, N, r);
        f3 rhs = (f + r - q.v * q.m) * q.sq;
        st3(scr, i, N, rhs);
        part += dot(rhs, rhs);
      });
#else
      auto vert = [&](int i, f3 sum, f3) {
        f3 rhs = vertex_body(i, sum);
        st3(scr, i, N, rhs);
        part += dot(rhs, rhs);
      };
#endif
      element_windows<THREADS, kFwdOpsPrecise>(S, lp, StagePlanar{xn, N}, vnow, fwd_tri_op(h, S.h64), fwd_bend_op(h, S.h64), vert);
      __syncthreads();
      PH(0)
      if (nself > 0 && !A.self_full) {
        if (self_friction_layers_lds<THREADS>(S, srec, b, rec_f, rec_r, lp, 3 * NP)) {
          const int M = srec.meta[(size_t) b * kMetaStride + kMetaStride - 1];
          const int *verts = srec.verts + (size_t) b * 2 * S.self_cap;
          for (int q = tid; q < M; q += THREADS) {
            const int i = verts[q];
            st3(scr, i, N, (ld3(rec_f, i, N) + ld3(rec_r, i, N) - ld3(vnow, i, N) * S.mass[i]) * S.sq_dinv[i]);
          }
          __syncthreads();
          self_done = true;
          part = 0.f;
        }
      }
      if constexpr (!H16) {
      const PlaneBuf tb0 = plane_buf(scr, N), tb1 = plane_buf(scr + N, N), tb2 = plane_buf(scr + 2 * N, N);
      for (int k0 = 0; k0 < VPT; k0 += 4) {
        float t[4][3];
#pragma unroll
        for (int j = 0; j < 4; j++) {
          const int i = tq + min(k0 + j, VPT - 1) * THREADS;
          t[j][0] = tb0.ld(i); t[j][1] = tb1.ld(i); t[j][2] = tb2.ld(i);
        }
#pragma unroll
        for (int j = 0; j < 4; j++) {
          if (k0 + j < VPT) {
            const int i = tq + (k0 + j) * THREADS;
            ((float2 *) lp)[i] = make_float2(t[j][0], t[j][1]); lp[2 * NP + i] = t[j][2];
            if (self_done) part += dot(mk(t[j][0], t[j][1], t[j][2]), mk(t[j][0], t[j][1], t[j][2]));
          }
        }
      }
      }
    } else {
      for (int t = tid; t < T; t += THREADS) {
        const int i0 = S.tri_v[t], i1 = S.tri_v[T + t], i2 = S.tri_v[2 * T + t];
        f3 r0, r1;
        const float4 D = S.tri_D[t];
        HybridTriOp{S.h64}(ld3(xn, i0, N), ld3(xn, i1, N), ld3(xn, i2, N), ld3(vnow, i0, N), ld3(vnow, i1, N), ld3(vnow, i2, N), D, S.tri_Dlo[t], S.tri_w2[t], r0, r1);
        f3 c1 = r0 * D.x + r1 * D.y, c2 = r0 * D.z + r1 * D.w;
        st3(corner, t, NC, mk(0, 0, 0) - c1 - c2); st3(corner, T + t, NC, c1); st3(corner, 2 * T + t, NC, c2);
      }
      for (int e = tid; e < E; e += THREADS) {
        const int i0 = S.bend_v[e], i1 = S.bend_v[E + e], i2 = S.bend_v[2 * E + e], i3 = S.bend_v[3 * E + e];
        const float4 w = S.bend_w[e];
        const float2 nw = S.bend_nw[e];
        f3 d;
        HybridBendOp{S.h64}(ld3(xn, i0, N), ld3(xn, i1, N), ld3(xn, i2, N), ld3(xn, i3, N), ld3(vnow, i0, N), ld3(vnow, i1, N), ld3(vnow, i2, N),
                            ld3(vnow, i3, N), w, S.bend_lo[e], nw.x, nw.y, d);
        const int base = 3 * T;
        st3(corner, base + e, NC, d * w.x); st3(corner, base + E + e, NC, d * w.y);
        st3(corner, base + 2 * E + e, NC, d * w.z); st3(corner, base + 3 * E + e, NC, d * w.w);
      }
      __syncthreads();
      PH(0)
      for (int i = tid; i < NP; i += THREADS) {
        f3 rhs = mk(0, 0, 0);
        if (i < N) {
          f3 fint = mk(0, 0, 0);
          const int k1 = S.inc_ptr[i + 1];
          for (int q = S.inc_ptr[i]; q < k1; q++) fint = fint + ld3(corner, S.inc_idx[q], NC);
          rhs = vertex_body(i, fint);
          part += dot(rhs, rhs);
        }
        ((float2 *) lp)[i] = make_float2(rhs.x, rhs.y); lp[2 * NP + i] = rhs.z;
      }
    }
    if (nself > 0 && !self_done) {
      __syncthreads();
      if (!self_friction_layers_lds<THREADS>(S, srec, b, rec_f, rec_r, lp, 3 * NP)) self_friction_layers<THREADS>(S, srec, b, rec_f, rec_r);
      part = 0.f;
      for (int i = tid; i < NP; i += THREADS) {
        f3 rhs = mk(0, 0, 0);
        if (i < N) rhs = (ld3(rec_f, i, N) + ld3(rec_r, i, N) - ld3(vnow, i, N) * S.mass[i]) * S.sq_dinv[i];
        if constexpr (H16) { if (i < N) st3(W.cg_r + off, i, N, rhs); }
        else { ((float2 *) lp)[i] = make_float2(rhs.x, rhs.y); lp[2 * NP + i] = rhs.z; }
        part += dot(rhs, rhs);
      }
      if constexpr (H16) __syncthreads();
    }
    float rr[VPT][3], ap[VPT][3], xx[XR > 0 ? XR : 1][3];
    if constexpr (H16) {
      const float *scr = W.cg_r + off;
      const PlaneBuf sb0 = plane_buf(scr, N), sb1 = plane_buf(scr + N, N), sb2 = plane_buf(scr + 2 * N, N);
      part = 0.f;
#pragma unroll
      for (int k = 0; k < VPT; k++) {
        const int i = tq + k * THREADS;
        rr[k][0] = sb0.ld(i); rr[k][1] = sb1.ld(i); rr[k][2] = sb2.ld(i);
      }
#pragma unroll
      for (int k = 0; k < VPT; k++) part = fmaf(rr[k][0], rr[k][0], fmaf(rr[k][1], rr[k][1], fmaf(rr[k][2], rr[k][2], part)));
    }
    double rz = block_sum<THREADS>((double) part, red);
    float hs = 1.f, pn = 0.f;
#pragma unroll
    for (int k = 0; k < VPT; k++) {
      const int i = tq + k * THREADS;
      if constexpr (!H16) {
        const float2 q = ((const float2 *) lp)[i];
        rr[k][0] = q.x; rr[k][1] = q.y; rr[k][2] = lp[2 * NP + i];
      }
#pragma unroll
      for (int c = 0; c < 3; c++) {
        if (k < XR) xx[k < XR ? k : 0][c] = 0.f;
        else lx[((k - XR) * 3 + c) * THREADS + tq] = 0.f;
      }
    }
    const double rz_b = rz;
    constexpr bool defl = DEFL;
    auto deflate = [&](double &rzv) {
      constexpr int DK = 16;
      float *scr = lp;
      const float4 DC_G *U4 = (const float4 DC_G *) S.defl_u;
      const float4 DC_G *AU4 = (const float4 DC_G *) S.defl_au;
      __syncthreads();
#pragma unroll 1
      for (int c = 0; c < 3; c++) {
        float acc[DK];
#pragma unroll
        for (int j = 0; j < DK; j++) acc[j] = 0.f;
#pragma unroll
        for (int k = 0; k < VPT; k++) {
          const int i = tq + k * THREADS;
          const float rv = c == 0 ? rr[k][0] : (c == 1 ? rr[k][1] : rr[k][2]);
#pragma unroll
          for (int q = 0; q < DK / 4; q++) {
            const float4 u = U4[(size_t) i * (DK / 4) + q];
            acc[4 * q] = fmaf(u.x, rv, acc[4 * q]); acc[4 * q + 1] = fmaf(u.y, rv, acc[4 * q + 1]);
            acc[4 * q + 2] = fmaf(u.z, rv, acc[4 * q + 2]); acc[4 * q + 3] = fmaf(u.w, rv, acc[4 * q + 3]);
          }
        }
#pragma unroll
        for (int j = 0; j < DK; j++) {
          const float v = wave_sum_f(acc[j]);
          if (lane == 0) scr[wv * 48 + c * DK + j] = v;
        }
      }
      __syncthreads();
      if (tid < 48) {
        float sacc = 0.f;
#pragma unroll
        for (int w = 0; w < WAVES; w++) sacc += scr[w * 48 + tid];
        scr[WAVES * 48 + tid] = sacc;
      }
      __syncthreads();
      if (tid < 48) {
        const int c = tid / DK, j = tid % DK;
        float sacc = 0.f;
#pragma unroll
        for (int l = 0; l < DK; l++) sacc = fmaf(S.defl_g[j * DK + l], scr[WAVES * 48 + c * DK + l], sacc);
        scr[WAVES * 48 + 48 + tid] = sacc;
// ... 351 lines not shown
```

diffcloth_amd/csrc/dc_tables.cpp:

```cpp
#include "dc_tables.h"
#include <algorithm>
#include <cmath>
#include <cstdlib>
#include <cstring>

namespace dc {

static float low_part(double v) { return (float) (v - (double) (float) v); }

void HostTables::build(const HostSystem &H, const dc_params &p, const TableSwitches &sw) {
  *this = HostTables();
  const int N = H.N, T = H.T, E = H.E, Af = (int) H.att_vertex.size();
  tri_v.resize(3 * (size_t) T); tri_D64.resize(4 * (size_t) T); tri_Dlo.resize(4 * (size_t) T);
  for (int t = 0; t < T; t++) {
    for (int k = 0; k < 3; k++) tri_v[(size_t) k * T + t] = H.tri[3 * t + k];
    for (int k = 0; k < 4; k++) { tri_D64[(size_t) k * T + t] = H.tri_D[4 * (size_t) t + k]; tri_Dlo[4 * (size_t) t + k] = low_part(H.tri_D[4 * (size_t) t + k]); }
  }
  bend_v.resize(4 * (size_t) E); bend_nw.resize(2 * (size_t) E); bend_w64.resize(4 * (size_t) E); bend_nw64.resize(2 * (size_t) E); bend_lo.resize(4 * (size_t) E);
  for (int e = 0; e < E; e++) {
    for (int k = 0; k < 4; k++) { bend_v[(size_t) k * E + e] = H.bend_v[4 * e + k]; bend_w64[(size_t) k * E + e] = H.bend_w[4 * (size_t) e + k]; }
    bend_nw[2 * e] = (float) H.bend_n[e]; bend_nw[2 * e + 1] = (float) H.bend_w2[e];
    bend_nw64[e] = H.bend_n[e]; bend_nw64[(size_t) E + e] = H.bend_w2[e];
    for (int k = 1; k < 4; k++) bend_lo[4 * (size_t) e + k - 1] = low_part(H.bend_w[4 * (size_t) e + k]);
    bend_lo[4 * (size_t) e + 3] = low_part(H.bend_n[e]);
  }
  dinv.resize(N);
  std::vector<double> diag(N, 0.0);
  for (int r = 0; r < N; r++)
    for (int k = H.P_ptr[r]; k < H.P_ptr[r + 1]; k++) {
      bandwidth = std::max(bandwidth, std::abs(H.P_col[k] - r));
      if (H.P_col[k] == r) diag[r] = H.P_val[k];
    }
  for (int r = 0; r < N; r++) dinv[r] = (float) (1.0 / diag[r]);
  att_of_vertex.assign(N, -1);
  for (int a = 0; a < Af; a++) att_of_vertex[H.att_vertex[a]] = a;
  {
    double mr = H.radii.empty() ? 0.0 : H.radii[0];
    for (double r : H.radii) mr = std::max(mr, r);
    max_radii = (float) mr;
    self_cap = std::min(p.max_self_contacts > 0 ? p.max_self_contacts : std::max(2048, N), 16000);
    self_lds = sw.self_lds ? 1 : 0;
  }
  {
    const int nchunks = (N + 63) / 64;
    ell_ptr.resize(nchunks); ell_w.resize(nchunks);
    for (int ch = 0; ch < nchunks; ch++) {
      int w = 0;
      for (int r = 64 * ch; r < std::min(N, 64 * ch + 64); r++) w = std::max(w, H.P_ptr[r + 1] - H.P_ptr[r]);
      ell_ptr[ch] = (int) (ell.size() / 2); ell_w[ch] = w;
      ell.resize(ell.size() + (size_t) 2 * 64 * w);
      for (int s = 0; s < w; s++)
        for (int l = 0; l < 64; l++) {
          const int r = 64 * ch + l;
          int col = std::min(r, N - 1);
          float val = 0.f;
          if (r < N && H.P_ptr[r] + s < H.P_ptr[r + 1]) { col = H.P_col[H.P_ptr[r] + s]; val = (float) H.P_val[H.P_ptr[r] + s]; }
          int bits;
          std::memcpy(&bits, &val, sizeof(int));
          const size_t o = 2 * ((size_t) ell_ptr[ch] + (size_t) s * 64 + l);
          ell[o] = col; ell[o + 1] = bits;
        }
    }
  }
  if (sw.windows && win.build(H, kWindowLdsBudget)) { win_ok = 1; nwin = win.nwin; }
  if (pk.build(H)) {
    pk_ok = 1; pk_vpt = pk.vpt; pk_threads = pk.threads;
    if (sw.pk_ofs && sw.pk_h16 && win_ok && (pk_threads == 768 || pk_vpt == 20)) { pk.to_offsets(); pk_ofs = 1; }
  } else {
    sq_dinv.assign((size_t) round64(N), 0.f);
    for (int r = 0; r < N; r++) if (diag[r] != 0.0) sq_dinv[r] = (float) (1.0 / std::sqrt(diag[r]));
  }
  defl_rows = win_ok ? (pk_ok ? pk_threads * pk_vpt : round64(N)) : 0;
  if (pk_ok && win_ok && dense.build(H, sw.dense_max_n)) dense_ld = dense.ld;
}

void HostTables::set_deflation(bool built, const TableSwitches &sw) {
  fwd_defl = (built && ((pk_ok && pk_threads == 512 && pk_vpt >= 4) || !pk_ok)) ? 1 : 0;
  adj_coarse = (built && sw.adj_coarse) ? 1 : 0;
}

}
```

diffcloth_amd/csrc/dc_tables.h:

```cpp
#pragma once
#include <vector>
#include "../../include/diffcloth_hip.h"
#include "dc_dense.h"
#include "dc_packets.h"
#include "dc_system.h"
#include "dc_windows.h"

namespace dc {

constexpr size_t kWindowLdsBudget = (size_t) 150 * 1024;

inline int round64(int v) { return (v + 63) / 64 * 64; }

struct TableSwitches {
  bool windows = true;
  int dense_max_n = 0;
  bool self_lds = true;
  bool adj_coarse = true;
  bool pk_h16 = true;
  bool pk_ofs = true;
};

struct HostTables {
  int bandwidth = 0;
  int win_ok = 0, nwin = 0;
  int pk_ok = 0, pk_vpt = 0, pk_threads = 0;
  int pk_ofs = 0;
  int defl_rows = 0;
  int fwd_defl = 0, adj_coarse = 0;
  int dense_ld = 0;
  int self_cap = 0, self_lds = 1;
  float max_radii = 0.f;

  std::vector<int> tri_v, bend_v;
  std::vector<float> bend_nw;
  std::vector<float> dinv;
  std::vector<int> att_of_vertex;
  std::vector<double> tri_D64, bend_w64, bend_nw64;
  std::vector<float> tri_Dlo, bend_lo;
  std::vector<int> ell;
  std::vector<int> ell_ptr, ell_w;
  std::vector<float> sq_dinv;
  HostWindows win;
  HostPackets pk;
  HostDense dense;

  void build(const HostSystem &H, const dc_params &p, const TableSwitches &sw);
  void set_deflation(bool built, const TableSwitches &sw);
};

}
```

diffcloth_amd/csrc/dc_windows.cpp:

```cpp
#include "dc_windows.h"
#include <algorithm>
#include <cstdlib>
#include <cstring>

namespace dc {

namespace {

inline int fbits(float v) { int b; std::memcpy(&b, &v, sizeof(int)); return b; }

struct Plan { int nwin = 0, vcap = 0, nrcap = 0; };

struct WinScan {
  std::vector<int> tris, bends;
  int lo = 0, hi = 0;
};

void scan_window(const HostSystem &H, int v0, int v1, WinScan &s) {
  s.tris.clear(); s.bends.clear();
  s.lo = v0; s.hi = v1;
  auto in = [&](int v) { return v >= v0 && v < v1; };
  for (int t = 0; t < H.T; t++) {
    const int *q = &H.tri[3 * t];
    if (in(q[0]) || in(q[1]) || in(q[2])) {
      s.tris.push_back(t);
      for (int k = 0; k < 3; k++) { s.lo = std::min(s.lo, q[k]); s.hi = std::max(s.hi, q[k] + 1); }
    }
  }
  for (int e = 0; e < H.E; e++) {
    const int *q = &H.bend_v[4 * e];
    if (in(q[0]) || in(q[1]) || in(q[2]) || in(q[3])) {
      s.bends.push_back(e);
      for (int k = 0; k < 4; k++) { s.lo = std::min(s.lo, q[k]); s.hi = std::max(s.hi, q[k] + 1); }
    }
  }
}

void order_by_first_use(const HostSystem &H, int v0, int v1, bool bends, std::vector<int> &list) {
  const int T = H.T, E = H.E;
  std::vector<char> placed(bends ? E : T, 0), member(bends ? E : T, 0);
  for (int id : list) member[id] = 1;
  std::vector<int> out;
  out.reserve(list.size());
  std::vector<std::vector<int>> inc(v1 - v0);
  size_t depth = 0;
  for (int v = v0; v < v1; v++) {
    for (int k = H.inc_ptr[v]; k < H.inc_ptr[v + 1]; k++) {
      const int idx = H.inc_idx[k];
      const bool is_bend = idx >= 3 * T;
      if (is_bend != bends) continue;
      const int id = is_bend ? (idx - 3 * T) % E : idx % T;
      if (member[id]) inc[v - v0].push_back(id);
    }
    depth = std::max(depth, inc[v - v0].size());
  }
  for (size_t j = 0; j < depth; j++)
    for (int v = v0; v < v1; v++)
      if (j < inc[v - v0].size()) {
        const int id = inc[v - v0][j];
        if (!placed[id]) { placed[id] = 1; out.push_back(id); }
      }
  for (int id : list)
    if (!placed[id]) out.push_back(id);
  list.swap(out);
}

Plan plan_for(const HostSystem &H, int own, const std::vector<int> &emin, const std::vector<int> &emax) {
  Plan p;
  p.nwin = (H.N + own - 1) / own;
  for (int w = 0; w < p.nwin; w++) {
    const int v0 = w * own, v1 = std::min(H.N, v0 + own);
    int lo = v0, hi = v1, nt = 0, nb = 0;
    auto in = [&](int v) { return v >= v0 && v < v1; };
    for (int t = 0; t < H.T; t++) {
      if (emax[t] < v0 || emin[t] >= v1) continue;
      const int *q = &H.tri[3 * t];
      if (in(q[0]) || in(q[1]) || in(q[2])) { nt++; lo = std::min(lo, emin[t]); hi = std::max(hi, emax[t] + 1); }
    }
    for (int e = 0; e < H.E; e++) {
      const int id = H.T + e;
      if (emax[id] < v0 || emin[id] >= v1) continue;
      const int *q = &H.bend_v[4 * e];
      if (in(q[0]) || in(q[1]) || in(q[2]) || in(q[3])) { nb++; lo = std::min(lo, emin[id]); hi = std::max(hi, emax[id] + 1); }
    }
    p.vcap = std::max(p.vcap, hi - lo);
    p.nrcap = std::max(p.nrcap, 2 * nt + nb + 1 + kWinDumpSlots);
  }
  return p;
}

}

bool HostWindows::build(const HostSystem &H, size_t lds_budget) {
  *this = HostWindows();
  const int N = H.N, T = H.T, E = H.E;
  if (N <= 0 || T <= 0) return false;
  std::vector<int> emin(T + E), emax(T + E);
  for (int t = 0; t < T; t++) {
    emin[t] = std::min({H.tri[3 * t], H.tri[3 * t + 1], H.tri[3 * t + 2]});
    emax[t] = std::max({H.tri[3 * t], H.tri[3 * t + 1], H.tri[3 * t + 2]});
  }
  for (int e = 0; e < E; e++) {
    const int *q = &H.bend_v[4 * e];
    emin[T + e] = std::min({q[0], q[1], q[2], q[3]});
    emax[T + e] = std::max({q[0], q[1], q[2], q[3]});
  }
  const int kmax = (N + 63) / 64;
  Plan best;
  int best_own = 0;
  for (int nw = 1; nw <= std::min(kmax, 64) && best_own == 0; nw++) {
    const int k = (kmax + nw - 1) / nw;
    if (nw > 1 && (kmax + nw - 2) / (nw - 1) == k) continue;
    Plan p = plan_for(H, 64 * k, emin, emax);
    const size_t bytes = sizeof(float) * ((size_t) 6 * p.vcap + (size_t) 3 * p.nrcap);
    if (bytes <= lds_budget && p.vcap <= 65535 && p.nrcap <= 32767) { best = p; best_own = 64 * k; }
  }
  if (best_own == 0) return false;
  if (best.nwin > 1 && best_own > 1024 && best_own % 1024 != 0) {
    const int rounded = best_own / 1024 * 1024;
    Plan p = plan_for(H, rounded, emin, emax);
    best = p; best_own = rounded;
  }
  return build_own(H, best_own);
}

bool HostWindows::build_own(const HostSystem &H, int own_size) {
  *this = HostWindows();
  const int N = H.N, T = H.T, E = H.E;
  if (N <= 0 || T <= 0 || own_size <= 0 || own_size % 64 != 0) return false;
  std::vector<int> emin(T + E), emax(T + E);
  for (int t = 0; t < T; t++) {
    emin[t] = std::min({H.tri[3 * t], H.tri[3 * t + 1], H.tri[3 * t + 2]});
    emax[t] = std::max({H.tri[3 * t], H.tri[3 * t + 1], H.tri[3 * t + 2]});
  }
  for (int e = 0; e < E; e++) {
    const int *q = &H.bend_v[4 * e];
    emin[T + e] = std::min({q[0], q[1], q[2], q[3]});
    emax[T + e] = std::max({q[0], q[1], q[2], q[3]});
  }
  const Plan best = plan_for(H, own_size, emin, emax);
  if (best.vcap > 65535 || best.nrcap > 32767) return false;
  const int best_own = own_size;
  own = best_own; nwin = best.nwin; vcap = best.vcap; nrcap = best.nrcap;
  lds_bytes = sizeof(float) * ((size_t) 6 * vcap + (size_t) 3 * nrcap);

  const int nchunks = (N + 63) / 64;
  inc_ptr.assign(nchunks, 0); inc_n.assign(nchunks, 0);
  std::vector<int> tri_local(T), bend_local(E);
  WinScan s;
  for (int w = 0; w < nwin; w++) {
    const int v0 = w * own, v1 = std::min(N, v0 + own);
    scan_window(H, v0, v1, s);
    static const bool reorder = !(getenv("DC_WIN_ORDER") && getenv("DC_WIN_ORDER")[0] == '0');
    if (reorder) {
      order_by_first_use(H, v0, v1, false, s.tris);
      order_by_first_use(H, v0, v1, true, s.bends);
    }
    const int ntri = (int) s.tris.size(), nbend = (int) s.bends.size();
    const int tri_off = (int) (tri_rec.size() / 4), bend_off = (int) (bend_rec.size() / 4);
    const int d[8] = {v0, v1, s.lo, s.hi - s.lo, tri_off, ntri, bend_off, nbend};
    win.insert(win.end(), d, d + 8);
    for (int k = 0; k < ntri; k++) {
      const int t = s.tris[k];
      tri_local[t] = k;
      const int j0 = H.tri[3 * t] - s.lo, j1 = H.tri[3 * t + 1] - s.lo, j2 = H.tri[3 * t + 2] - s.lo;
      const int r[4] = {j0 | (j1 << 16), j2, fbits((float) H.tri_w2[t]), t};
      tri_rec.insert(tri_rec.end(), r, r + 4);
      for (int q = 0; q < 4; q++) tri_D.push_back((float) H.tri_D[4 * t + q]);
      for (int q = 0; q < 4; q++) tri_Dlo.push_back((float) (H.tri_D[4 * t + q] - (double) (float) H.tri_D[4 * t + q]));
    }
    for (int k = 0; k < nbend; k++) {
      const int e = s.bends[k];
      bend_local[e] = k;
      const int *q = &H.bend_v[4 * e];
      const int r[4] = {(q[0] - s.lo) | ((q[1] - s.lo) << 16), (q[2] - s.lo) | ((q[3] - s.lo) << 16), fbits((float) H.bend_n[e]),
                        fbits((float) H.bend_w2[e])};
      bend_rec.insert(bend_rec.end(), r, r + 4);
      for (int c = 0; c < 4; c++) bend_w.push_back((float) H.bend_w[4 * e + c]);
      for (int c = 1; c < 4; c++) bend_lo.push_back((float) (H.bend_w[4 * e + c] - (double) (float) H.bend_w[4 * e + c]));
      bend_lo.push_back((float) (H.bend_n[e] - (double) (float) H.bend_n[e]));
    }
    const int zero_slot = 2 * ntri + nbend;
    for (int ch = v0 / 64; ch < (v1 + 63) / 64; ch++) {
      std::vector<std::vector<int>> codes(64);
      std::vector<std::vector<std::pair<int, float>>> rows(64);
      int wt = 0, wb = 0;
      for (int l = 0; l < 64; l++) {
        const int v = 64 * ch + l;
        if (v >= v1) break;
        for (int k = H.inc_ptr[v]; k < H.inc_ptr[v + 1]; k++) {
          const int idx = H.inc_idx[k];
          if (idx < 3 * T) {
            const int corner = idx / T, t = idx % T;
            const int p0 = tri_local[t], p1 = ntri + tri_local[t];
            if (corner == 1) codes[l].push_back(p0 << 1);
            else if (corner == 2) codes[l].push_back(p1 << 1);
            else { codes[l].push_back((p0 << 1) | 1); codes[l].push_back((p1 << 1) | 1); }
          } else {
            const int corner = (idx - 3 * T) / E, e = (idx - 3 * T) % E;
            rows[l].push_back({2 * ntri + bend_local[e], (float) H.bend_w[4 * e + corner]});
          }
        }
        wt = std::max(wt, (int) codes[l].size());
        wb = std::max(wb, (int) rows[l].size());
      }
      const int nt4 = std::max(1, (wt + 7) / 8);
      const int nb4 = std::max(2, ((wb + 1) / 2 + 1) / 2 * 2);
      inc_ptr[ch] = (int) (inc.size() / 4); inc_n[ch] = nb4 | (nt4 << 16);
      const size_t base = inc.size();
      inc.resize(base + (size_t) 4 * 64 * (nt4 + nb4), 0);
      for (int l = 0; l < 64; l++) {
        for (int k = 0; k < 8 * nt4; k++) {
          const int code = k < (int) codes[l].size() ? codes[l][k] : (zero_slot << 1);
          const size_t o = base + 4 * ((size_t) (k / 8) * 64 + l) + (k % 8) / 2;
          inc[o] |= (k % 2) ? (code << 16) : code;
        }
        for (size_t k = 0; k < rows[l].size(); k++) {
          const size_t o = base + 4 * ((size_t) (nt4 + k / 2) * 64 + l) + 2 * (k % 2);
          inc[o] = rows[l][k].first; inc[o + 1] = fbits(rows[l][k].second);
        }
        for (size_t k = rows[l].size(); k < (size_t) 2 * nb4; k++) {
          const size_t o = base + 4 * ((size_t) (nt4 + k / 2) * 64 + l) + 2 * (k % 2);
          inc[o] = zero_slot; inc[o + 1] = 0;
        }
      }
    }
  }
  ok = true;
  return true;
}

}
```

diffcloth_amd/csrc/dc_windows.h:

```cpp
#pragma once
#include <cstddef>
#include <vector>
#include "dc_system.h"

namespace dc {

constexpr int kWinDumpSlots = 64;

struct HostWindows {
  bool ok = false;
  int own = 0;
  int nwin = 0;
  int vcap = 0;
  int nrcap = 0;
  size_t lds_bytes = 0;
  std::vector<int> win;
  std::vector<int> tri_rec;
  std::vector<float> tri_D;
  std::vector<int> bend_rec;
  std::vector<float> bend_w;
  std::vector<float> tri_Dlo, bend_lo;
  std::vector<int> inc;
  std::vector<int> inc_ptr, inc_n;

  bool build(const HostSystem &H, size_t lds_budget);
  bool build_own(const HostSystem &H, int own_size);
};

}
```

diffcloth_amd/csrc/dc_winlib.h:

```cpp
#pragma once
#include <type_traits>
#include "dc_devlib.h"

namespace dc {

struct WinLds {
  float2 *a1xy, *a2xy, *erxy;
  float *a1z, *a2z, *erz;
};

template <class TB>
__device__ __forceinline__ WinLds win_lds(const TB &S, float *lds) {
  const int vc = S.win_vcap, nr = S.win_nrcap;
  WinLds L;
  L.a1xy = (float2 *) lds; L.a2xy = (float2 *) (lds + 2 * vc); L.erxy = (float2 *) (lds + 4 * vc);
  L.a1z = lds + 4 * vc + 2 * nr; L.a2z = L.a1z + vc; L.erz = L.a2z + vc;
  return L;
}

__device__ __forceinline__ f3 ldw(const float2 *xy, const float *z, int j) { const float2 q = xy[j]; return mk(q.x, q.y, z[j]); }
__device__ __forceinline__ void stw(float2 *xy, float *z, int j, f3 v) { xy[j] = make_float2(v.x, v.y); z[j] = v.z; }

struct In2Plain {
  const float *__restrict__ v;
  int N;
  __device__ __forceinline__ f3 operator()(int i) const { return mk(v[i], v[N + i], v[2 * N + i]); }
};
#ifndef DC_WIN_EB
#define DC_WIN_EB 4
#endif
constexpr int kWinMaxBatch = DC_WIN_EB;
#ifndef DC_WIN_SUB1024
#define DC_WIN_SUB1024 1
#endif
constexpr int kWinSubBatch1024 = DC_WIN_SUB1024;
#ifndef DC_WIN_LEGACY1024
#define DC_WIN_LEGACY1024 1
#endif
constexpr bool kWinLegacy1024 = DC_WIN_LEGACY1024 != 0;
#ifdef DC_WIN_NOFENCE
#define DC_WIN_GATHER_FENCE
#else
#define DC_WIN_GATHER_FENCE if constexpr (SUB > 1) __builtin_amdgcn_sched_barrier(0);
#endif
template <int B, class F>
__device__ __forceinline__ void batch_exact(int take, F f) {
  if constexpr (B <= 1) f(std::integral_constant<int, 1>());
  else {
    if (take >= B) f(std::integral_constant<int, B>());
    else batch_exact<B - 1>(take, f);
  }
}
template <int MAXB, class F>
__device__ __forceinline__ int batch_dispatch(int left, F f) {
  const int take = left >= 2 * MAXB ? MAXB : (left > MAXB ? (left + 1) / 2 : left);
  batch_exact<MAXB>(take, f);
  return take;
}

#ifdef DC_PROFILE_PHASES
static __device__ long long g_win_ph[4];
#define WPH_DECL long long wph_t = clock64();
#define WPH(k) { if (blockIdx.x == 0 && threadIdx.x == 0) { long long n_ = clock64(); g_win_ph[k] += n_ - wph_t; wph_t = n_; } }
#else
#define WPH_DECL
#define WPH(k)
#endif

template <class V, class = void> struct vert_has_pre : std::false_type {};
template <class V> struct vert_has_pre<V, std::void_t<decltype(std::declval<V &>().pre(0))>> : std::true_type {};
template <class P, class O, bool NOA = false>
struct VertWithPre {
  static constexpr bool kIgnoresInput1 = NOA;
  P p; O o;
  __device__ __forceinline__ auto pre(int i) { return p(i); }
  template <class Q> __device__ __forceinline__ void operator()(int i, f3 sum, f3 a, const Q &q) { o(i, sum, a, q); }
};
template <class P, class O> __device__ __forceinline__ VertWithPre<P, O> vert_with_pre(P p, O o) { return VertWithPre<P, O>{p, o}; }
template <class P, class O> __device__ __forceinline__ VertWithPre<P, O, true> vert_with_pre_noa(P p, O o) { return VertWithPre<P, O, true>{p, o}; }
template <class O>
struct VertNoA {
  static constexpr bool kIgnoresInput1 = true;
  O o;
  __device__ __forceinline__ void operator()(int i, f3 sum, f3 a) { o(i, sum, a); }
};
template <class O> __device__ __forceinline__ VertNoA<O> vert_noa(O o) { return VertNoA<O>{o}; }
template <class V, class = void> struct vert_ignores_a : std::false_type {};
template <class V> struct vert_ignores_a<V, std::enable_if_t<V::kIgnoresInput1>> : std::true_type {};

template <int EB, bool PRECISE>
struct WinTriRecs { int4 r[EB]; float4 D[EB]; float4 Dl[PRECISE ? EB : 1]; };
template <int EB, bool PRECISE>
struct WinBendRecs { int4 r[EB]; float4 w[EB]; float4 wl[PRECISE ? EB : 1]; };

template <int THREADS, bool PRECISE = false, class TB, class Stage1, class In2, class TriOp, class BendOp, class VertOp>
__device__ __forceinline__ void element_windows_t(const TB &S, int w0, int w1, float *lds, Stage1 stage1,
                                                  In2 in2, TriOp tri_op, BendOp bend_op, VertOp vert_op) {
  const int tid = threadIdx.x, lane = tid & 63;
  const WinLds L = win_lds(S, lds);
  constexpr int MB = kWinMaxBatch;
  constexpr int VPB = 6;
  constexpr bool PAIR = THREADS < 1024;
  for (int w = w0; w < w1; w++) {
    const int4 d0 = S.win[2 * w], d1 = S.win[2 * w + 1];
    const int v0 = d0.x, v1 = d0.y, lo = d0.z, vs = d0.w, toff = d1.x, nt = d1.y, boff = d1.z, nb = d1.w;
    WPH_DECL
    auto tri_load = [&](auto nc, WinTriRecs<MB, PRECISE> &R, int t0) {
#pragma unroll
      for (int j = 0; j < decltype(nc)::value; j++) {
        const int t = min(t0 + j * THREADS, nt - 1);
        R.r[j] = S.wtri_rec[toff + t]; R.D[j] = S.wtri_D[toff + t];
        if constexpr (PRECISE) R.Dl[j] = S.wtri_Dlo[toff + t];
      }
    };
    auto bend_load = [&](auto nc, WinBendRecs<MB, PRECISE> &R, int e0) {
#pragma unroll
      for (int j = 0; j < decltype(nc)::value; j++) {
        const int e = min(e0 + j * THREADS, nb - 1);
        R.r[j] = S.wbend_rec[boff + e]; R.w[j] = S.wbend_w[boff + e];
        if constexpr (PRECISE) R.wl[j] = S.wbend_lo[boff + e];
      }
    };
    WinTriRecs<MB, PRECISE> tcur;
    WinBendRecs<MB, PRECISE> bcur;
    const int dump = 2 * nt + nb + 1 + lane;
    constexpr bool NOA = vert_ignores_a<VertOp>::value;
    if (!NOA || w == w0) __syncthreads();
    constexpr int SVR = THREADS < 1024 ? 3 : 2;
    for (int j0 = tid; j0 < vs; j0 += SVR * THREADS) {
      f3 u[SVR], sv[SVR];
#pragma unroll
      for (int q = 0; q < SVR; q++) {
        const int j = j0 + q * THREADS, i = lo + (j < vs ? j : j0);
        u[q] = in2(i); sv[q] = stage1(i);
      }
#pragma unroll
      for (int q = 0; q < SVR; q++) {
        const int j = j0 + q * THREADS;
        if (q == 0 || j < vs) { stw(L.a2xy, L.a2z, j, u[q]); stw(L.a1xy, L.a1z, j, sv[q]); }
      }
    }
    __syncthreads();
    if (tid == 0) stw(L.erxy, L.erz, 2 * nt + nb, mk(0, 0, 0));
    WPH(0)
    constexpr int SUBMAX = THREADS >= 1024 ? kWinSubBatch1024 : MB;
    auto tri_compute = [&](auto ebc, const WinTriRecs<MB, PRECISE> &R, int t0) {
      constexpr int EB = decltype(ebc)::value;
      constexpr int SUB = EB < SUBMAX ? EB : SUBMAX;
      if constexpr (SUBMAX == 1 && kWinLegacy1024) {
#pragma unroll
        for (int j = 0; j < EB; j++) {
          const int t = t0 + j * THREADS;
          const int j0 = R.r[j].x & 0xffff, j1 = (int) ((unsigned) R.r[j].x >> 16), j2 = R.r[j].y;
          f3 r0, r1;
          if constexpr (PRECISE)
            tri_op(ldw(L.a1xy, L.a1z, j0), ldw(L.a1xy, L.a1z, j1), ldw(L.a1xy, L.a1z, j2), ldw(L.a2xy, L.a2z, j0),
                   ldw(L.a2xy, L.a2z, j1), ldw(L.a2xy, L.a2z, j2), R.D[j], R.Dl[j], __int_as_float(R.r[j].z), r0, r1);
          else
            tri_op(ldw(L.a1xy, L.a1z, j0), ldw(L.a1xy, L.a1z, j1), ldw(L.a1xy, L.a1z, j2), ldw(L.a2xy, L.a2z, j0),
                   ldw(L.a2xy, L.a2z, j1), ldw(L.a2xy, L.a2z, j2), R.D[j], __int_as_float(R.r[j].z), r0, r1);
          if (t < nt) { stw(L.erxy, L.erz, t, r0 * R.D[j].x + r1 * R.D[j].y); stw(L.erxy, L.erz, nt + t, r0 * R.D[j].z + r1 * R.D[j].w); }
        }
      } else
#pragma unroll
      for (int s0 = 0; s0 < EB; s0 += SUB) {
        f3 ea0[SUB], ea1[SUB], eb0[SUB], eb1[SUB];
#pragma unroll
        for (int u = 0; u < SUB; u++) {
          const int j = min(s0 + u, EB - 1);
          const int j0 = R.r[j].x & 0xffff, j1 = (int) ((unsigned) R.r[j].x >> 16), j2 = R.r[j].y;
          const f3 p0 = ldw(L.a1xy, L.a1z, j0), p1 = ldw(L.a1xy, L.a1z, j1), p2 = ldw(L.a1xy, L.a1z, j2);
          const f3 q0 = ldw(L.a2xy, L.a2z, j0), q1 = ldw(L.a2xy, L.a2z, j1), q2 = ldw(L.a2xy, L.a2z, j2);
          ea0[u] = p1 - p0; ea1[u] = p2 - p0; eb0[u] = q1 - q0; eb1[u] = q2 - q0;
        }
        DC_WIN_GATHER_FENCE
        f3 c1[SUB], c2[SUB];
#pragma unroll
        for (int u = 0; u < SUB; u++) {
          const int j = min(s0 + u, EB - 1);
          f3 r0, r1;
          if constexpr (PRECISE) tri_op.edges(ea0[u], ea1[u], eb0[u], eb1[u], R.D[j], R.Dl[j], __int_as_float(R.r[j].z), r0, r1);
          else tri_op.edges(ea0[u], ea1[u], eb0[u], eb1[u], R.D[j], __int_as_float(R.r[j].z), r0, r1);
          c1[u] = r0 * R.D[j].x + r1 * R.D[j].y; c2[u] = r0 * R.D[j].z + r1 * R.D[j].w;
        }
#pragma unroll
        for (int u = 0; u < SUB; u++) {
          if (s0 + u < EB) {
            const int t = t0 + (s0 + u) * THREADS;
            const bool live = t < nt;
            stw(L.erxy, L.erz, live ? t : dump, c1[u]);
            stw(L.erxy, L.erz, live ? nt + t : dump, c2[u]);
          }
        }
      }
    };
    auto bend_compute = [&](auto ebc, const WinBendRecs<MB, PRECISE> &R, int e0) {
      constexpr int EB = decltype(ebc)::value;
      constexpr int SUB = EB < SUBMAX ? EB : SUBMAX;
      if constexpr (SUBMAX == 1 && kWinLegacy1024) {
#pragma unroll
        for (int j = 0; j < EB; j++) {
          const int e = e0 + j * THREADS;
          const int j0 = R.r[j].x & 0xffff, j1 = (int) ((unsigned) R.r[j].x >> 16), j2 = R.r[j].y & 0xffff, j3 = (int) ((unsigned) R.r[j].y >> 16);
          f3 res;
          if constexpr (PRECISE)
            bend_op(ldw(L.a1xy, L.a1z, j0), ldw(L.a1xy, L.a1z, j1), ldw(L.a1xy, L.a1z, j2), ldw(L.a1xy, L.a1z, j3),
                    ldw(L.a2xy, L.a2z, j0), ldw(L.a2xy, L.a2z, j1), ldw(L.a2xy, L.a2z, j2), ldw(L.a2xy, L.a2z, j3), R.w[j], R.wl[j],
                    __int_as_float(R.r[j].z), __int_as_float(R.r[j].w), res);
          else
            bend_op(ldw(L.a1xy, L.a1z, j0), ldw(L.a1xy, L.a1z, j1), ldw(L.a1xy, L.a1z, j2), ldw(L.a1xy, L.a1z, j3),
                    ldw(L.a2xy, L.a2z, j0), ldw(L.a2xy, L.a2z, j1), ldw(L.a2xy, L.a2z, j2), ldw(L.a2xy, L.a2z, j3), R.w[j],
                    __int_as_float(R.r[j].z), __int_as_float(R.r[j].w), res);
          if (e < nb) stw(L.erxy, L.erz, 2 * nt + e, res);
        }
      } else
#pragma unroll
      for (int s0 = 0; s0 < EB; s0 += SUB) {
        f3 ea1[SUB], ea2[SUB], ea3[SUB], eb1[SUB], eb2[SUB], eb3[SUB];
#pragma unroll
        for (int u = 0; u < SUB; u++) {
          const int j = min(s0 + u, EB - 1);
          const int j0 = R.r[j].x & 0xffff, j1 = (int) ((unsigned) R.r[j].x >> 16), j2 = R.r[j].y & 0xffff, j3 = (int) ((unsigned) R.r[j].y >> 16);
          const f3 p0 = ldw(L.a1xy, L.a1z, j0), q0 = ldw(L.a2xy, L.a2z, j0);
          ea1[u] = ldw(L.a1xy, L.a1z, j1) - p0; ea2[u] = ldw(L.a1xy, L.a1z, j2) - p0; ea3[u] = ldw(L.a1xy, L.a1z, j3) - p0;
          eb1[u] = ldw(L.a2xy, L.a2z, j1) - q0; eb2[u] = ldw(L.a2xy, L.a2z, j2) - q0; eb3[u] = ldw(L.a2xy, L.a2z, j3) - q0;
        }
        DC_WIN_GATHER_FENCE
        f3 res[SUB];
#pragma unroll
        for (int u = 0; u < SUB; u++) {
          const int j = min(s0 + u, EB - 1);
          if constexpr (PRECISE)
            bend_op.edges(ea1[u], ea2[u], ea3[u], eb1[u], eb2[u], eb3[u], R.w[j], R.wl[j], __int_as_float(R.r[j].z), __int_as_float(R.r[j].w), res[u]);
          else
            bend_op.edges(ea1[u], ea2[u], ea3[u], eb1[u], eb2[u], eb3[u], R.w[j], __int_as_float(R.r[j].z), __int_as_float(R.r[j].w), res[u]);
        }
#pragma unroll
        for (int u = 0; u < SUB; u++) {
          if (s0 + u < EB) {
            const int e = e0 + (s0 + u) * THREADS;
            stw(L.erxy, L.erz, e < nb ? 2 * nt + e : dump, res[u]);
          }
        }
      }
    };
    const int wbase = (SUBMAX == 1 && kWinLegacy1024) ? 0 : __builtin_amdgcn_readfirstlane(tid & ~63);
    for (int q = 0, rounds = max(nt - wbase + THREADS - 1, 0) / THREADS; q < rounds;) {
      const int left = rounds - q, t0 = q * THREADS + tid;
      q += batch_dispatch<MB>(left, [&](auto ebc) { tri_load(ebc, tcur, t0); tri_compute(ebc, tcur, t0); });
    }
    WPH(1)
    for (int q = 0, rounds = max(nb - wbase + THREADS - 1, 0) / THREADS; q < rounds;) {
      const int left = rounds - q, e0 = q * THREADS + tid;
      q += batch_dispatch<MB>(left, [&](auto ebc) { bend_load(ebc, bcur, e0); bend_compute(ebc, bcur, e0); });
    }
    __syncthreads();
    WPH(2)
    auto gather_tri = [&](const int4 &w, bool live, float &sx, float &sy, float &sz) {
      const int wd[4] = {w.x, w.y, w.z, w.w};
      const int one = live ? 0x3f800000 : 0;
#pragma unroll
      for (int e = 0; e < 8; e++) {
        const int code = (e & 1) ? (int) ((unsigned) wd[e >> 1] >> 16) : (wd[e >> 1] & 0xffff);
        const float c = __int_as_float(one | ((code & 1) << 31));
        const float2 q = L.erxy[code >> 1];
        const float z = L.erz[code >> 1];
        sx = fmaf(c, q.x, sx); sy = fmaf(c, q.y, sy); sz = fmaf(c, z, sz);
      }
    };
    auto gather = [&](const int4 (&e)[VPB], int s0, int np, float &sx, float &sy, float &sz) {
#pragma unroll
      for (int j = 0; j < VPB; j++) {
        const float on = (s0 + j < np) ? 1.f : 0.f;
        const float2 qa = L.erxy[e[j].x], qb = L.erxy[e[j].z];
        const float za = L.erz[e[j].x], zb = L.erz[e[j].z];
        const float ca = __int_as_float(e[j].y) * on, cb = __int_as_float(e[j].w) * on;
        sx = fmaf(ca, qa.x, sx); sy = fmaf(ca, qa.y, sy); sz = fmaf(ca, za, sz);
        sx = fmaf(cb, qb.x, sx); sy = fmaf(cb, qb.y, sy); sz = fmaf(cb, zb, sz);
      }
    };
    for (int i = v0 + tid; i < v1; i += (PAIR ? 2 : 1) * THREADS) {
      const int cha = __builtin_amdgcn_readfirstlane(i >> 6);
      const int na = S.winc_n[cha], nta = na >> 16, nba = na & 0xffff;
      const int4 DC_G *rowa = S.winc + S.winc_ptr[cha] + lane;
      const int4 DC_G *frowa = rowa + nta * 64;
      float ax = 0.f, ay = 0.f, az = 0.f;
      if constexpr (PAIR) {
        const int ib = i + THREADS;
        const bool vb = ib < v1;
        const int chb = __builtin_amdgcn_readfirstlane((vb ? ib : i) >> 6);
        const int nb_ = S.winc_n[chb], ntb = nb_ >> 16, nbb = nb_ & 0xffff;
        const int4 DC_G *rowb = S.winc + S.winc_ptr[chb] + lane;
        const int4 DC_G *frowb = rowb + ntb * 64;
        float bx = 0.f, by = 0.f, bz = 0.f;
        auto prea = [&]() { if constexpr (vert_has_pre<VertOp>::value) return vert_op.pre(i); else return 0; }();
        auto preb = [&]() { if constexpr (vert_has_pre<VertOp>::value) return vert_op.pre(vb ? ib : i); else return 0; }();
        {
          const int4 ta = rowa[0], tb = rowb[0];
          const int4 ta1 = rowa[min(1, nta - 1) * 64], tb1 = rowb[min(1, ntb - 1) * 64];
          int4 ea[VPB], eb[VPB];
#pragma unroll
          for (int j = 0; j < VPB; j++) { ea[j] = frowa[min(j, nba - 1) * 64]; eb[j] = frowb[min(j, nbb - 1) * 64]; }
          gather_tri(ta, true, ax, ay, az);
          gather_tri(tb, true, bx, by, bz);
          if (max(nta, ntb) > 1) {
            gather_tri(ta1, nta > 1, ax, ay, az);
            gather_tri(tb1, ntb > 1, bx, by, bz);
          }
          gather(ea, 0, nba, ax, ay, az);
          gather(eb, 0, nbb, bx, by, bz);
        }
        for (int s0 = 2; s0 < max(nta, ntb); s0++) {
          const int4 ta = rowa[min(s0, nta - 1) * 64], tb = rowb[min(s0, ntb - 1) * 64];
          gather_tri(ta, s0 < nta, ax, ay, az);
          gather_tri(tb, s0 < ntb, bx, by, bz);
        }
        for (int s0 = VPB; s0 < max(nba, nbb); s0 += VPB) {
          int4 ea[VPB], eb[VPB];
#pragma unroll
          for (int j = 0; j < VPB; j++) { ea[j] = frowa[min(s0 + j, nba - 1) * 64]; eb[j] = frowb[min(s0 + j, nbb - 1) * 64]; }
          gather(ea, s0, nba, ax, ay, az);
          gather(eb, s0, nbb, bx, by, bz);
        }
        if constexpr (vert_has_pre<VertOp>::value) {
          vert_op(i, mk(ax, ay, az), ldw(L.a1xy, L.a1z, i - lo), prea);
          if (vb) vert_op(ib, mk(bx, by, bz), ldw(L.a1xy, L.a1z, ib - lo), preb);
        } else {
          vert_op(i, mk(ax, ay, az), ldw(L.a1xy, L.a1z, i - lo));
          if (vb) vert_op(ib, mk(bx, by, bz), ldw(L.a1xy, L.a1z, ib - lo));
        }
      } else {
        auto prea = [&]() { if constexpr (vert_has_pre<VertOp>::value) return vert_op.pre(i); else return 0; }();
        {
          const int4 ta = rowa[0], ta1 = rowa[min(1, nta - 1) * 64];
          int4 ea[VPB];
#pragma unroll
          for (int j = 0; j < VPB; j++) ea[j] = frowa[min(j, nba - 1) * 64];
          gather_tri(ta, true, ax, ay, az);
          if (nta > 1) gather_tri(ta1, true, ax, ay, az);
          gather(ea, 0, nba, ax, ay, az);
        }
        for (int s0 = 2; s0 < nta; s0++) gather_tri(rowa[s0 * 64], true, ax, ay, az);
        for (int s0 = VPB; s0 < nba; s0 += VPB) {
          int4 ea[VPB];
#pragma unroll
          for (int j = 0; j < VPB; j++) ea[j] = frowa[min(s0 + j, nba - 1) * 64];
          gather(ea, s0, nba, ax, ay, az);
        }
        if constexpr (vert_has_pre<VertOp>::value) vert_op(i, mk(ax, ay, az), ldw(L.a1xy, L.a1z, i - lo), prea);
        else vert_op(i, mk(ax, ay, az), ldw(L.a1xy, L.a1z, i - lo));
      }
    }
    WPH(3)
  }
}

template <int THREADS, bool PRECISE = false, class Stage1, class TriOp, class BendOp, class VertOp>
__device__ __forceinline__ void element_windows(const DevSystem &S, float *lds, Stage1 stage1,
                                                const float *__restrict__ in2, TriOp tri_op, BendOp bend_op, VertOp vert_op) {
  element_windows_t<THREADS, PRECISE>(S, 0, S.nwin, lds, stage1, In2Plain{in2, S.N}, tri_op, bend_op, vert_op);
}

struct StagePlanar {
  const float *v;
  int N;
  __device__ __forceinline__ f3 operator()(int i) const { return mk(v[i], v[N + i], v[2 * N + i]); }
};

struct FwdTriOp {
  float h;
  __device__ __forceinline__ void operator()(f3 x0, f3 x1, f3 x2, f3 v0, f3 v1, f3 v2, float4 D, float w2, f3 &r0, f3 &r1) const {
    edges(x1 - x0, x2 - x0, v1 - v0, v2 - v0, D, w2, r0, r1);
  }
  __device__ __forceinline__ void edges(f3 a0, f3 a1, f3 b0, f3 b1, float4 D, float w2, f3 &r0, f3 &r1) const {
    f3 e0 = a0 + b0 * h, e1 = a1 + b1 * h;
    f3 f0 = e0 * D.x + e1 * D.z, f1 = e0 * D.y + e1 * D.w;
    Polar P = polar3x2(f0, f1);
    const float s = h * w2;
    r0 = (P.t0 - f0) * s; r1 = (P.t1 - f1) * s;
  }
};
struct FwdBendOp {
  float h;
  __device__ __forceinline__ void operator()(f3 x0, f3 x1, f3 x2, f3 x3, f3 v0, f3 v1, f3 v2, f3 v3, float4 w, float n, float w2, f3 &res) const {
    edges(x1 - x0, x2 - x0, x3 - x0, v1 - v0, v2 - v0, v3 - v0, w, n, w2, res);
  }
  __device__ __forceinline__ void edges(f3 a1, f3 a2, f3 a3, f3 b1, f3 b2, f3 b3, float4 w, float n, float w2, f3 &res) const {
    f3 ev = (a1 + b1 * h) * w.y;
    ev = ev + (a2 + b2 * h) * w.z;
    ev = ev + (a3 + b3 * h) * w.w;
    f3 p = mk(0, 0, 0);
    if (n > 1e-6f) p = normalized_fast(ev) * n;
    res = (p - ev) * (h * w2);
  }
};

struct PreciseTriOp {
  double h;
  __device__ __forceinline__ void operator()(f3 x0, f3 x1, f3 x2, f3 v0, f3 v1, f3 v2, float4 D, float4 Dl, float w2, f3 &r0, f3 &r1) const {
    edges(x1 - x0, x2 - x0, v1 - v0, v2 - v0, D, Dl, w2, r0, r1);
  }
  __device__ __forceinline__ void edges(f3 a0, f3 a1, f3 b0, f3 b1, float4 D, float4 Dl, float w2, f3 &r0, f3 &r1) const {
    const double e0x = (double) a0.x + h * (double) b0.x, e0y = (double) a0.y + h * (double) b0.y, e0z = (double) a0.z + h * (double) b0.z;
    const double e1x = (double) a1.x + h * (double) b1.x, e1y = (double) a1.y + h * (double) b1.y, e1z = (double) a1.z + h * (double) b1.z;
    const double Dx = (double) D.x + (double) Dl.x, Dy = (double) D.y + (double) Dl.y, Dz = (double) D.z + (double) Dl.z, Dw = (double) D.w + (double) Dl.w;
    const double f0x = e0x * Dx + e1x * Dz, f0y = e0y * Dx + e1y * Dz, f0z = e0z * Dx + e1z * Dz;
    const double f1x = e0x * Dy + e1x * Dw, f1y = e0y * Dy + e1y * Dw, f1z = e0z * Dy + e1z * Dw;
    const double a = f0x * f0x + f0y * f0y + f0z * f0z, b = f0x * f1x + f0y * f1y + f0z * f1z, c = f1x * f1x + f1y * f1y + f1z * f1z;
    const double s = sqrt(fmax(a * c - b * b, 1e-300)), t = sqrt(a + c + 2.0 * s), inv = 1.0 / (t * s);
    const double i00 = (c + s) * inv, i01 = -b * inv, i11 = (a + s) * inv;
    const double sc = h * (double) w2;
    r0 = mk((float) ((f0x * i00 + f1x * i01 - f0x) * sc), (float) ((f0y * i00 + f1y * i01 - f0y) * sc), (float) ((f0z * i00 + f1z * i01 - f0z) * sc));
    r1 = mk((float) ((f0x * i01 + f1x * i11 - f1x) * sc), (float) ((f0y * i01 + f1y * i11 - f1y) * sc), (float) ((f0z * i01 + f1z * i11 - f1z) * sc));
  }
};
struct PreciseBendOp {
  double h;
  __device__ __forceinline__ void operator()(f3 x0, f3 x1, f3 x2, f3 x3, f3 v0, f3 v1, f3 v2, f3 v3, float4 w, float4 wl, float n, float w2, f3 &res) const {
    edges(x1 - x0, x2 - x0, x3 - x0, v1 - v0, v2 - v0, v3 - v0, w, wl, n, w2, res);
  }
  __device__ __forceinline__ void edges(f3 a1, f3 a2, f3 a3, f3 b1, f3 b2, f3 b3, float4 w, float4 wl, float n, float w2, f3 &res) const {
    const double w1 = (double) w.y + (double) wl.x, w2d = (double) w.z + (double) wl.y, w3 = (double) w.w + (double) wl.z;
    const double ex = ((double) a1.x + h * (double) b1.x) * w1 + ((double) a2.x + h * (double) b2.x) * w2d + ((double) a3.x + h * (double) b3.x) * w3;
    const double ey = ((double) a1.y + h * (double) b1.y) * w1 + ((double) a2.y + h * (double) b2.y) * w2d + ((double) a3.y + h * (double) b3.y) * w3;
    const double ez = ((double) a1.z + h * (double) b1.z) * w1 + ((double) a2.z + h * (double) b2.z) * w2d + ((double) a3.z + h * (double) b3.z) * w3;
    double fac = -1.0;
    if (n > 1e-6f) {
      const double nn = (double) n + (double) wl.w, len = sqrt(ex * ex + ey * ey + ez * ez);
      fac = len > 0.0 ? nn / len - 1.0 : 0.0;
    }
    const double sc = fac * h * (double) w2;
    res = mk((float) (ex * sc), (float) (ey * sc), (float) (ez * sc));
  }
};

struct HybridTriOp {
  double h;
  __device__ __forceinline__ void operator()(f3 x0, f3 x1, f3 x2, f3 v0, f3 v1, f3 v2, float4 D, float4 Dl, float w2, f3 &r0, f3 &r1) const {
    edges(x1 - x0, x2 - x0, v1 - v0, v2 - v0, D, Dl, w2, r0, r1);
  }
  __device__ __forceinline__ void edges(f3 a0, f3 a1, f3 b0, f3 b1, float4 D, float4 Dl, float w2, f3 &r0, f3 &r1) const {
    const double e0x = (double) a0.x + h * (double) b0.x, e0y = (double) a0.y + h * (double) b0.y, e0z = (double) a0.z + h * (double) b0.z;
    const double e1x = (double) a1.x + h * (double) b1.x, e1y = (double) a1.y + h * (double) b1.y, e1z = (double) a1.z + h * (double) b1.z;
    const double Dx = (double) D.x + (double) Dl.x, Dy = (double) D.y + (double) Dl.y, Dz = (double) D.z + (double) Dl.z, Dw = (double) D.w + (double) Dl.w;
    const double f0x = e0x * Dx + e1x * Dz, f0y = e0y * Dx + e1y * Dz, f0z = e0z * Dx + e1z * Dz;
    const double f1x = e0x * Dy + e1x * Dw, f1y = e0y * Dy + e1y * Dw, f1z = e0z * Dy + e1z * Dw;
    const float e00 = (float) (f0x * f0x + f0y * f0y + f0z * f0z - 1.0), e01 = (float) (f0x * f1x + f0y * f1y + f0z * f1z),
                e11 = (float) (f1x * f1x + f1y * f1y + f1z * f1z - 1.0);
    const f3 f0 = mk((float) f0x, (float) f0y, (float) f0z), f1 = mk((float) f1x, (float) f1y, (float) f1z);
    const float trE = e00 + e11, q = trE + (e00 * e11 - e01 * e01);
    const float sm1 = q * fast_rcp(fast_sqrt(fmaxf(1.f + q, 1e-30f)) + 1.f);
    const float t = fast_sqrt(fmaxf(4.f + trE + 2.f * sm1, 1e-30f));
    const float tm2 = (trE + 2.f * sm1) * fast_rcp(t + 2.f);
    const float c = sm1 - tm2, it = fast_rcp(t);
    const float a = (e00 + c) * it, b = e01 * it, d = (e11 + c) * it;
    const float idet = fast_rcp((1.f + a) * (1.f + d) - b * b);
    const float m00 = (a + (a * d - b * b)) * idet, m01 = b * idet, m11 = (d + (a * d - b * b)) * idet;
    const float sc = -(float) h * w2;
    r0 = (f0 * m00 + f1 * m01) * sc; r1 = (f0 * m01 + f1 * m11) * sc;
  }
};
struct HybridBendOp {
  double h;
  __device__ __forceinline__ void operator()(f3 x0, f3 x1, f3 x2, f3 x3, f3 v0, f3 v1, f3 v2, f3 v3, float4 w, float4 wl, float n, float w2, f3 &res) const {
    edges(x1 - x0, x2 - x0, x3 - x0, v1 - v0, v2 - v0, v3 - v0, w, wl, n, w2, res);
  }
  __device__ __forceinline__ void edges(f3 a1, f3 a2, f3 a3, f3 b1, f3 b2, f3 b3, float4 w, float4 wl, float n, float w2, f3 &res) const {
    const double w1 = (double) w.y + (double) wl.x, w2d = (double) w.z + (double) wl.y, w3 = (double) w.w + (double) wl.z;
    const double ex = ((double) a1.x + h * (double) b1.x) * w1 + ((double) a2.x + h * (double) b2.x) * w2d + ((double) a3.x + h * (double) b3.x) * w3;
    const double ey = ((double) a1.y + h * (double) b1.y) * w1 + ((double) a2.y + h * (double) b2.y) * w2d + ((double) a3.y + h * (double) b3.y) * w3;
    const double ez = ((double) a1.z + h * (double) b1.z) * w1 + ((double) a2.z + h * (double) b2.z) * w2d + ((double) a3.z + h * (double) b3.z) * w3;
    float fac = -1.f;
    if (n > 1e-6f) {
      const double nn = (double) n + (double) wl.w, l2 = ex * ex + ey * ey + ez * ez;
      const float diff = (float) (nn * nn - l2), len = fast_sqrt((float) l2);
      fac = len > 0.f ? diff * fast_rcp(len * ((float) nn + len)) : 0.f;
    }
    const float sc = fac * (float) h * w2;
    res = mk((float) ex * sc, (float) ey * sc, (float) ez * sc);
  }
};

#ifndef DC_ELEMENT_OPS
#define DC_ELEMENT_OPS 1
#endif
#if DC_ELEMENT_OPS == 0
constexpr bool kFwdOpsPrecise = false;
__device__ __forceinline__ FwdTriOp fwd_tri_op(float h, double) { return FwdTriOp{h}; }
__device__ __forceinline__ FwdBendOp fwd_bend_op(float h, double) { return FwdBendOp{h}; }
#elif DC_ELEMENT_OPS == 2
constexpr bool kFwdOpsPrecise = true;
__device__ __forceinline__ PreciseTriOp fwd_tri_op(float, double h) { return PreciseTriOp{h}; }
__device__ __forceinline__ PreciseBendOp fwd_bend_op(float, double h) { return PreciseBendOp{h}; }
#else
constexpr bool kFwdOpsPrecise = true;
__device__ __forceinline__ HybridTriOp fwd_tri_op(float, double h) { return HybridTriOp{h}; }
__device__ __forceinline__ HybridBendOp fwd_bend_op(float, double h) { return HybridBendOp{h}; }
#endif

struct AdjTriOp {
  float h2;
  __device__ __forceinline__ void operator()(f3 q0, f3 q1, f3 q2, f3 x0, f3 x1, f3 x2, float4 D, float w2, f3 &r0, f3 &r1) const {
    edges(q1 - q0, q2 - q0, x1 - x0, x2 - x0, D, w2, r0, r1);
  }
  __device__ __forceinline__ void edges(f3 d0, f3 d1, f3 e0, f3 e1, float4 D, float w2, f3 &r0, f3 &r1) const {
    Polar P = polar3x2(e0 * D.x + e1 * D.z, e0 * D.y + e1 * D.w);
    f3 y0 = d0 * D.x + d1 * D.z, y1 = d0 * D.y + d1 * D.w;
    const float c = (dot(P.t1, y0) - dot(P.t0, y1)) * fast_rcp(P.trS);
    f3 z0 = y0 * P.i00 + y1 * P.i01, z1 = y0 * P.i01 + y1 * P.i11;
    z0 = z0 - P.t0 * dot(P.t0, z0) - P.t1 * dot(P.t1, z0);
    z1 = z1 - P.t0 * dot(P.t0, z1) - P.t1 * dot(P.t1, z1);
    const float s = h2 * w2;
    r0 = (y0 - (P.t1 * c + z0)) * s; r1 = (y1 - (z1 - P.t0 * c)) * s;
// ... 22 lines not shown
```

include/diffcloth_hip.h:

```cpp
#ifndef DIFFCLOTH_HIP_H
#define DIFFCLOTH_HIP_H

#ifdef __cplusplus
extern "C" {
#endif

typedef struct dc_ctx dc_ctx;

enum { DC_OK = 0, DC_ERR_INVALID = 1, DC_ERR_HIP = 2, DC_ERR_STATE = 3, DC_ERR_TOPOLOGY = 4, DC_ERR_CAPACITY = 5 };

enum { DC_PRIM_SPHERE = 0, DC_PRIM_CAPSULE = 1, DC_PRIM_PLANE = 2, DC_PRIM_BOWL = 3,
       DC_PRIM_SPHERE_DISCRETIZED = 4    };

typedef struct dc_primitive {
  int kind;
  int group;
  double center[3];
  double top_offset[3];
  double corner2[3];
  double radius;
  double length;
  double mu;
  int rotates;
} dc_primitive;

typedef struct dc_params {
  double time_step;
  double density;
  double k_stretch, k_bend, k_att;
  double gravity[3];
  double forward_tol;
  double backward_tol;
  int gravity_enabled, contact_enabled, selfcollision_enabled;
  int gradient_clipping;
  double gradient_clipping_threshold;
  int pd_iter_cap;
  int adjoint_iter_cap;
  double cg_rel_tol;
  int cg_max_iter;
  int stall_window;
  int adjoint_mode;
  double adjoint_rel_tol;
  int adjoint_block_precond;
  int adjoint_fp32_only;
  int max_self_contacts;
  int forward_deflation;
} dc_params;

typedef struct dc_step_stats {
  int converged;
  int pd_iters;
  int cg_iters;
  int prim_contacts;
  int self_contacts;
  float last_xdiff;
  int self_overflow;
} dc_step_stats;

typedef struct dc_bwd_stats {
  int converged;
  int adjoint_iters;
  int cg_iters;
  int clipped;
  int used_direct;
  float last_udiff;
  int refine_cycles;
  int fp64_iters;
  int residual_verified;
  int workgroups;
} dc_bwd_stats;

int dc_create(int device_id, dc_ctx **out);
int dc_destroy(dc_ctx *ctx);
const char *dc_last_error(const dc_ctx *ctx);
const char *dc_version(void);

int dc_set_mesh(dc_ctx *ctx, int num_vertices, const double *rest_pos , int num_triangles, const int *tris );
int dc_set_attachments(dc_ctx *ctx, int num_fixed, const int *vertex );
int dc_set_params(dc_ctx *ctx, const dc_params *p);
int dc_set_primitives(dc_ctx *ctx, int count, const dc_primitive *prims);
int dc_build(dc_ctx *ctx);
void dc_default_params(dc_params *p);
int dc_set_solver(dc_ctx *ctx, double forward_tol, double backward_tol, int gradient_clipping, double clip_threshold,
                  int force_direct_adjoint);
int dc_set_flags(dc_ctx *ctx, int gravity_enabled, int contact_enabled, int selfcollision_enabled);

int dc_get_counts(const dc_ctx *ctx, int *out6);
int dc_get_system_matrix(const dc_ctx *ctx, int *row_ptr , int *col , double *val );
int dc_get_vertex_data(const dc_ctx *ctx, double *mass, double *area, double *radii);

int dc_alloc_batch(dc_ctx *ctx, int batch, int tape_steps);
int dc_set_state(dc_ctx *ctx, int slot, const double *x , const double *v );
int dc_get_state(dc_ctx *ctx, int slot, double *x, double *v);
int dc_set_mu(dc_ctx *ctx, const double *mu);
int dc_set_uniform_force(dc_ctx *ctx, const double *f);
int dc_set_vertex_forces(dc_ctx *ctx, const double *f );
int dc_set_vertex_force_field(dc_ctx *ctx, const double *f );

int dc_step_forward(dc_ctx *ctx, int slot, const double *fixed_pts, dc_step_stats *stats);
int dc_get_record(dc_ctx *ctx, int slot, double *f, double *r);
int dc_get_contacts(dc_ctx *ctx, int slot, int *prim_group, double *normal);

int dc_get_self_contacts(dc_ctx *ctx, int slot, int rollout, int cap, int *count, int *num_layers, int *pairs ,
                         int *layer , double *normal );

typedef struct dc_record {
  const double *x, *v;
  const double *f;
  const double *r;
  const int *prim;
  const double *normal;
  const double *x_fixed;
  const int *self_count;
  const int *self_pairs;
  const int *self_layer;
  const double *self_normal;
  const double *self_d;
} dc_record;
int dc_set_record(dc_ctx *ctx, int slot, const dc_record *rec);

int dc_step_backward(dc_ctx *ctx, int slot, const double *dL_dxnew, const double *dL_dvnew,
                     const double *dL_dxinit, const double *dL_dvinit, int is_start, double *dL_dx,
                     double *dL_dv, double *dL_dxfixed, double *dL_dmu, dc_bwd_stats *stats);

int dc_get_param_gradients(dc_ctx *ctx, int slot, double *out );
int dc_get_force_gradient(dc_ctx *ctx, double *dL_df );
int dc_keep_force_gradients(dc_ctx *ctx, int keep);
int dc_get_force_gradients(dc_ctx *ctx, int slot0, int nslots, double *dL_df );

int dc_use_stream(dc_ctx *ctx, void *hip_stream);
int dc_set_state_dev(dc_ctx *ctx, int slot, const void *d_x , const void *d_v , int is_f32);
int dc_get_state_dev(dc_ctx *ctx, int slot, void *d_x , void *d_v , int is_f32);
int dc_step_forward_dev(dc_ctx *ctx, int slot, const void *d_fixed_pts , int is_f32);
int dc_step_backward_dev(dc_ctx *ctx, int slot, const void *d_dL_dxnew, const void *d_dL_dvnew, const void *d_dL_dxinit ,
                         const void *d_dL_dvinit , int is_start, void *d_dL_dx, void *d_dL_dv, void *d_dL_dxfixed ,
                         void *d_dL_dmu , int is_f32);

int dc_rollout_forward(dc_ctx *ctx, int slot, int nsteps);
int dc_seed_gradient(dc_ctx *ctx, int slot, const double *target , double scale_x);
int dc_rollout_backward(dc_ctx *ctx, int slot, int nsteps);
int dc_get_gradient(dc_ctx *ctx, double *dL_dx, double *dL_dv, double *dL_dmu );
int dc_set_gradient(dc_ctx *ctx, const double *dL_dx , const double *dL_dv );

int dc_set_fixed_point_schedule(dc_ctx *ctx, int slot0, int nsteps, const double *xf );
int dc_set_force_schedule(dc_ctx *ctx, int slot0, int nsteps, const double *fu , const double *fv_scale );
int dc_set_seed_schedule(dc_ctx *ctx, int slot0, int nslots, const double *dL_dx , const double *dL_dv );
int dc_clear_schedules(dc_ctx *ctx);
int dc_get_states(dc_ctx *ctx, int slot0, int nslots, double *x, double *v);
int dc_get_dxfixed(dc_ctx *ctx, int slot0, int nslots, double *dL_dxfixed );
int dc_set_trajectory_start(dc_ctx *ctx, int start_slot);
int dc_get_stats(dc_ctx *ctx, int slot, dc_step_stats *fwd , dc_bwd_stats *bwd );
int dc_sync(dc_ctx *ctx);
int dc_get_cluster(const dc_ctx *ctx, int *workgroups_per_rollout, int *rollouts_per_launch);
int dc_get_self_friction_path(dc_ctx *ctx, int *out , int reset);
int dc_get_layout(const dc_ctx *ctx, int *out6);
int dc_get_packet_layout(const dc_ctx *ctx, int *byte_offsets);
int dc_get_deflation(const dc_ctx *ctx, int *vectors, int *probe_iterations);

int dc_comm_unique_id(char *id128 );
int dc_comm_init(dc_ctx *ctx, int nranks, int rank, const char *id128);
int dc_allreduce_sum(dc_ctx *ctx, double *inout, int count);
int dc_comm_destroy(dc_ctx *ctx);
int dc_timer_start(dc_ctx *ctx);
int dc_timer_stop(dc_ctx *ctx, float *ms);
int dc_kernel_times(dc_ctx *ctx, float *fwd_ms, int *fwd_launches, float *bwd_ms, int *bwd_launches, int reset);
int dc_get_adjoint_matrix(dc_ctx *ctx, int slot, int rollout, double *K );
int dc_dense_phase_times(dc_ctx *ctx, float *ms3, int reset);

#ifdef __cplusplus
}
#endif
#endif
```

Baseline: 9995.

## Precompute flat-bending stiffness as sparse vertex rows in element windows

When every bending flap is flat, the bending contribution becomes a constant linear operator, so it is assembled on the host into a per-vertex sparse row matrix scaled by h^2. The windowed element kernel then drops the bend-element stage and gathers the precomputed row coefficients against vertex differences, and the forward RHS adds the bend term from those rows. This replaces per-step bend element evaluation with a cheaper row gather and shrinks LDS use. In exchange it adds an extra sync per window, a serial double-precision CSR loop per vertex in RHS assembly, and it only applies when the rest shape is flat.

Result: faster. 11020, median of 6 (+10.2%).

```diff
diff --git a/diffcloth_amd/capi.py b/diffcloth_amd/capi.py
--- a/diffcloth_amd/capi.py
+++ b/diffcloth_amd/capi.py
@@ -53,7 +53,7 @@
     "dc_step_forward", "dc_get_record", "dc_get_contacts", "dc_get_self_contacts", "dc_step_backward", "dc_rollout_forward",
     "dc_seed_gradient", "dc_rollout_backward", "dc_get_gradient", "dc_get_param_gradients", "dc_get_stats", "dc_sync", "dc_timer_start",
     "dc_timer_stop", "dc_kernel_times", "dc_get_cluster", "dc_set_gradient", "dc_set_fixed_point_schedule", "dc_set_force_schedule",
-    "dc_set_seed_schedule", "dc_clear_schedules", "dc_get_states", "dc_get_dxfixed", "dc_get_layout", "dc_get_packet_layout", "dc_comm_unique_id", "dc_comm_init", "dc_allreduce_sum", "dc_comm_destroy",
+    "dc_set_seed_schedule", "dc_clear_schedules", "dc_get_states", "dc_get_dxfixed", "dc_get_layout", "dc_get_packet_layout", "dc_get_bend_rows", "dc_comm_unique_id", "dc_comm_init", "dc_allreduce_sum", "dc_comm_destroy",
     "dc_get_deflation", "dc_set_record", "dc_set_trajectory_start", "dc_keep_force_gradients", "dc_get_force_gradients", "dc_use_stream", "dc_set_state_dev", "dc_get_state_dev", "dc_step_forward_dev", "dc_step_backward_dev",
     "dc_get_self_friction_path", "dc_get_adjoint_matrix", "dc_dense_phase_times",
 ]
@@ -446,6 +446,11 @@
         self._chk(self.lib.dc_get_packet_layout(self.h, C.byref(k)))
         return bool(k.value)
 
+    def bend_rows(self):
+        k = C.c_int()
+        self._chk(self.lib.dc_get_bend_rows(self.h, C.byref(k)))
+        return bool(k.value)
+
     def deflation(self):
         k = C.c_int(); pi = C.c_int()
         self._chk(self.lib.dc_get_deflation(self.h, C.byref(k), C.byref(pi)))
diff --git a/diffcloth_amd/csrc/dc_device.h b/diffcloth_amd/csrc/dc_device.h
--- a/diffcloth_amd/csrc/dc_device.h
+++ b/diffcloth_amd/csrc/dc_device.h
@@ -73,7 +73,11 @@
   const int DC_C *winc_ptr;
   const int DC_C *winc_n;
   int nwin, win_vcap, win_nrcap, win_ok;
-  int win_lds_bytes, pad2;
+  int win_lds_bytes;
+  int win_rows;
+  const int DC_G *brow_ptr;
+  const int DC_G *brow_col;
+  const double DC_G *brow_val;
   const float DC_G *radii;
   const int DC_G *conn_ptr;
   const int DC_G *conn_idx;
diff --git a/diffcloth_amd/csrc/dc_engine.hip b/diffcloth_amd/csrc/dc_engine.hip
--- a/diffcloth_amd/csrc/dc_engine.hip
+++ b/diffcloth_amd/csrc/dc_engine.hip
@@ -252,7 +252,7 @@
 
 static void set_decisions(DevSystem &S, const HostTables &plan) {
   S.win_ok = plan.win_ok; S.nwin = plan.nwin; S.pk_ok = plan.pk_ok; S.pk_vpt = plan.pk_vpt; S.pk_threads = plan.pk_threads;
-  S.pk_ofs = plan.pk_ofs;
+  S.pk_ofs = plan.pk_ofs; S.win_rows = plan.bend_rows;
   S.fwd_defl = plan.fwd_defl; S.adj_coarse = plan.adj_coarse; S.dense_ld = plan.dense_ld;
   S.max_radii = plan.max_radii; S.self_cap = plan.self_cap; S.self_lds = plan.self_lds;
 }
@@ -601,6 +601,7 @@
   sw.adj_coarse = adj_coarse;
   sw.pk_h16 = pk_h16_enabled() != 0;
   sw.pk_ofs = env_not_off("DC_PK_OFS", true);
+  sw.bend_rows = env_not_off("DC_BEND_ROWS", true);
   HostTables plan;
   plan.build(H, p, sw);
   HostDeflation *HD = nullptr;
@@ -669,6 +670,11 @@
     if ((rc = upload_as<int>(c, &S.winc, HW.inc))) return rc;
     if ((rc = upload<int>(c, &S.winc_ptr, HW.inc_ptr))) return rc;
     if ((rc = upload<int>(c, &S.winc_n, HW.inc_n))) return rc;
+    if (HW.rows) {
+      if ((rc = upload<int>(c, &S.brow_ptr, HW.brow_ptr))) return rc;
+      if ((rc = upload<int>(c, &S.brow_col, HW.brow_col))) return rc;
+      if ((rc = upload<double>(c, &S.brow_val, HW.brow_val))) return rc;
+    }
     S.win_vcap = HW.vcap; S.win_nrcap = HW.nrcap; S.win_lds_bytes = (int) HW.lds_bytes;
   }
   if (plan.pk_ok) {
@@ -1413,6 +1419,13 @@
   return DC_OK;
 }
 
+int dc_get_bend_rows(const dc_ctx *c, int *rows) {
+  if (!c || !rows) return DC_ERR_INVALID;
+  if (!c->built) return DC_ERR_STATE;
+  *rows = c->S.win_rows;
+  return DC_OK;
+}
+
 int dc_get_layout(const dc_ctx *c, int *out6) {
   if (!c || !out6) return DC_ERR_INVALID;
   if (!c->built) return DC_ERR_STATE;
diff --git a/diffcloth_amd/csrc/dc_forward_pk_kernel.h b/diffcloth_amd/csrc/dc_forward_pk_kernel.h
--- a/diffcloth_amd/csrc/dc_forward_pk_kernel.h
+++ b/diffcloth_amd/csrc/dc_forward_pk_kernel.h
@@ -82,7 +82,20 @@
     if (A.fv2) fext = fext + ld3(A.fv2 + off, i, N);
     f3 v0 = v + fext * (h / m);
     st3(vnow, i, N, v0);
-    st3(g, i, N, v0 * m);
+    f3 gi = v0 * m;
+    if (S.win_rows) {
+      const f3 xi = ld3(xn, i, N);
+      double bx = 0, by = 0, bz = 0;
+      const int k1 = S.brow_ptr[i + 1];
+      for (int k = S.brow_ptr[i]; k < k1; k++) {
+        const f3 xj = ld3(xn, S.brow_col[k], N);
+        const double c = S.brow_val[k];
+        bx += c * ((double) xj.x - (double) xi.x); by += c * ((double) xj.y - (double) xi.y); bz += c * ((double) xj.z - (double) xi.z);
+      }
+      const double ih = -1.0 / S.h64;
+      gi = gi + mk((float) (ih * bx), (float) (ih * by), (float) (ih * bz));
+    }
+    st3(g, i, N, gi);
     part += dot(v0, v0);
     int prim = -1;
     f3 nrm = mk(0, 0, 0);
@@ -153,7 +166,7 @@
         part += dot(rhs, rhs);
       };
 #endif
-      element_windows<THREADS, kFwdOpsPrecise>(S, lp, StagePlanar{xn, N}, vnow, fwd_tri_op(h, S.h64), fwd_bend_op(h, S.h64), vert);
+      element_windows<THREADS, kFwdOpsPrecise, 2, -1>(S, lp, StagePlanar{xn, N}, vnow, fwd_tri_op(h, S.h64), fwd_bend_op(h, S.h64), vert);
       __syncthreads();
       PH(0)
       if (nself > 0 && !A.self_full) {
diff --git a/diffcloth_amd/csrc/dc_tables.cpp b/diffcloth_amd/csrc/dc_tables.cpp
--- a/diffcloth_amd/csrc/dc_tables.cpp
+++ b/diffcloth_amd/csrc/dc_tables.cpp
@@ -62,7 +62,7 @@
         }
     }
   }
-  if (sw.windows && win.build(H, kWindowLdsBudget)) { win_ok = 1; nwin = win.nwin; }
+  if (sw.windows && win.build(H, kWindowLdsBudget, sw.bend_rows, p.time_step)) { win_ok = 1; nwin = win.nwin; bend_rows = win.rows ? 1 : 0; }
   if (pk.build(H)) {
     pk_ok = 1; pk_vpt = pk.vpt; pk_threads = pk.threads;
     if (sw.pk_ofs && sw.pk_h16 && win_ok && (pk_threads == 768 || pk_vpt == 20)) { pk.to_offsets(); pk_ofs = 1; }
diff --git a/diffcloth_amd/csrc/dc_tables.h b/diffcloth_amd/csrc/dc_tables.h
--- a/diffcloth_amd/csrc/dc_tables.h
+++ b/diffcloth_amd/csrc/dc_tables.h
@@ -19,12 +19,14 @@
   bool adj_coarse = true;
   bool pk_h16 = true;
   bool pk_ofs = true;
+  bool bend_rows = true;
 };
 
 struct HostTables {
   int bandwidth = 0;
   int win_ok = 0, nwin = 0;
   int pk_ok = 0, pk_vpt = 0, pk_threads = 0;
+  int bend_rows = 0;
   int pk_ofs = 0;
   int defl_rows = 0;
   int fwd_defl = 0, adj_coarse = 0;
diff --git a/diffcloth_amd/csrc/dc_windows.cpp b/diffcloth_amd/csrc/dc_windows.cpp
--- a/diffcloth_amd/csrc/dc_windows.cpp
+++ b/diffcloth_amd/csrc/dc_windows.cpp
@@ -2,6 +2,7 @@
 #include <algorithm>
 #include <cstdlib>
 #include <cstring>
+#include <map>
 
 namespace dc {
 
@@ -9,7 +10,7 @@
 
 inline int fbits(float v) { int b; std::memcpy(&b, &v, sizeof(int)); return b; }
 
-struct Plan { int nwin = 0, vcap = 0, nrcap = 0; };
+struct Plan { int nwin = 0, vcap = 0, nrcap = 0, nrcap_rows = 0; };
 
 struct WinScan {
   std::vector<int> tris, bends;
@@ -85,13 +86,34 @@
     }
     p.vcap = std::max(p.vcap, hi - lo);
     p.nrcap = std::max(p.nrcap, 2 * nt + nb + 1 + kWinDumpSlots);
+    p.nrcap_rows = std::max(p.nrcap_rows, 2 * nt + 1 + kWinDumpSlots);
   }
   return p;
 }
 
-}
-
-bool HostWindows::build(const HostSystem &H, size_t lds_budget) {
+bool all_flaps_flat(const HostSystem &H) {
+  if (H.E <= 0) return false;
+  for (int e = 0; e < H.E; e++)
+    if (!((float) H.bend_n[e] <= 1e-6f)) return false;
+  return true;
+}
+
+std::vector<std::map<int, double>> bend_matrix_rows(const HostSystem &H) {
+  std::vector<std::map<int, double>> B(H.N);
+  for (int e = 0; e < H.E; e++) {
+    const int *q = &H.bend_v[4 * e];
+    const double *w = &H.bend_w[4 * (size_t) e];
+    const double ew[4] = {-(w[1] + w[2] + w[3]), w[1], w[2], w[3]};
+    for (int c = 0; c < 4; c++)
+      for (int d = 0; d < 4; d++)
+        if (q[d] != q[c]) B[q[c]][q[d]] += H.bend_w2[e] * w[c] * ew[d];
+  }
+  return B;
+}
+
+}
+
+bool HostWindows::build(const HostSystem &H, size_t lds_budget, bool want_rows, double h) {
   *this = HostWindows();
   const int N = H.N, T = H.T, E = H.E;
   if (N <= 0 || T <= 0) return false;
@@ -121,10 +143,10 @@
     Plan p = plan_for(H, rounded, emin, emax);
     best = p; best_own = rounded;
   }
-  return build_own(H, best_own);
-}
-
-bool HostWindows::build_own(const HostSystem &H, int own_size) {
+  return build_own(H, best_own, want_rows, h);
+}
+
+bool HostWindows::build_own(const HostSystem &H, int own_size, bool want_rows, double h) {
   *this = HostWindows();
   const int N = H.N, T = H.T, E = H.E;
   if (N <= 0 || T <= 0 || own_size <= 0 || own_size % 64 != 0) return false;
@@ -141,7 +163,17 @@
   const Plan best = plan_for(H, own_size, emin, emax);
   if (best.vcap > 65535 || best.nrcap > 32767) return false;
   const int best_own = own_size;
-  own = best_own; nwin = best.nwin; vcap = best.vcap; nrcap = best.nrcap;
+  rows = want_rows && all_flaps_flat(H);
+  own = best_own; nwin = best.nwin; vcap = best.vcap; nrcap = rows ? best.nrcap_rows : best.nrcap;
+  std::vector<std::map<int, double>> B;
+  if (rows) {
+    B = bend_matrix_rows(H);
+    brow_ptr.assign(N + 1, 0);
+    for (int v = 0; v < N; v++) {
+      for (const auto &jc : B[v]) { brow_col.push_back(jc.first); brow_val.push_back(h * h * jc.second); }
+      brow_ptr[v + 1] = (int) brow_col.size();
+    }
+  }
   lds_bytes = sizeof(float) * ((size_t) 6 * vcap + (size_t) 3 * nrcap);
 
   const int nchunks = (N + 63) / 64;
@@ -156,6 +188,7 @@
       order_by_first_use(H, v0, v1, false, s.tris);
       order_by_first_use(H, v0, v1, true, s.bends);
     }
+    if (rows) s.bends.clear();
     const int ntri = (int) s.tris.size(), nbend = (int) s.bends.size();
     const int tri_off = (int) (tri_rec.size() / 4), bend_off = (int) (bend_rec.size() / 4);
     const int d[8] = {v0, v1, s.lo, s.hi - s.lo, tri_off, ntri, bend_off, nbend};
@@ -183,7 +216,7 @@
     const int zero_slot = 2 * ntri + nbend;
     for (int ch = v0 / 64; ch < (v1 + 63) / 64; ch++) {
       std::vector<std::vector<int>> codes(64);
-      std::vector<std::vector<std::pair<int, float>>> rows(64);
+      std::vector<std::vector<std::pair<int, float>>> vrows(64);
       int wt = 0, wb = 0;
       for (int l = 0; l < 64; l++) {
         const int v = 64 * ch + l;
@@ -196,13 +229,15 @@
             if (corner == 1) codes[l].push_back(p0 << 1);
             else if (corner == 2) codes[l].push_back(p1 << 1);
             else { codes[l].push_back((p0 << 1) | 1); codes[l].push_back((p1 << 1) | 1); }
-          } else {
+          } else if (!rows) {
             const int corner = (idx - 3 * T) / E, e = (idx - 3 * T) % E;
-            rows[l].push_back({2 * ntri + bend_local[e], (float) H.bend_w[4 * e + corner]});
+            vrows[l].push_back({2 * ntri + bend_local[e], (float) H.bend_w[4 * e + corner]});
           }
         }
+        if (rows)
+          for (int k = brow_ptr[v]; k < brow_ptr[v + 1]; k++) vrows[l].push_back({brow_col[k] - s.lo, (float) brow_val[k]});
         wt = std::max(wt, (int) codes[l].size());
-        wb = std::max(wb, (int) rows[l].size());
+        wb = std::max(wb, (int) vrows[l].size());
       }
       const int nt4 = std::max(1, (wt + 7) / 8);
       const int nb4 = std::max(2, ((wb + 1) / 2 + 1) / 2 * 2);
@@ -215,13 +250,14 @@
           const size_t o = base + 4 * ((size_t) (k / 8) * 64 + l) + (k % 8) / 2;
           inc[o] |= (k % 2) ? (code << 16) : code;
         }
-        for (size_t k = 0; k < rows[l].size(); k++) {
+        for (size_t k = 0; k < vrows[l].size(); k++) {
           const size_t o = base + 4 * ((size_t) (nt4 + k / 2) * 64 + l) + 2 * (k % 2);
-          inc[o] = rows[l][k].first; inc[o + 1] = fbits(rows[l][k].second);
-        }
-        for (size_t k = rows[l].size(); k < (size_t) 2 * nb4; k++) {
+          inc[o] = vrows[l][k].first; inc[o + 1] = fbits(vrows[l][k].second);
+        }
+        const int pad = rows ? std::min(64 * ch + l, v1 - 1) - s.lo : zero_slot;
+        for (size_t k = vrows[l].size(); k < (size_t) 2 * nb4; k++) {
           const size_t o = base + 4 * ((size_t) (nt4 + k / 2) * 64 + l) + 2 * (k % 2);
-          inc[o] = zero_slot; inc[o + 1] = 0;
+          inc[o] = pad; inc[o + 1] = 0;
         }
       }
     }
diff --git a/diffcloth_amd/csrc/dc_windows.h b/diffcloth_amd/csrc/dc_windows.h
--- a/diffcloth_amd/csrc/dc_windows.h
+++ b/diffcloth_amd/csrc/dc_windows.h
@@ -22,9 +22,12 @@
   std::vector<float> tri_Dlo, bend_lo;
   std::vector<int> inc;
   std::vector<int> inc_ptr, inc_n;
+  bool rows = false;
+  std::vector<int> brow_ptr, brow_col;
+  std::vector<double> brow_val;
 
-  bool build(const HostSystem &H, size_t lds_budget);
-  bool build_own(const HostSystem &H, int own_size);
+  bool build(const HostSystem &H, size_t lds_budget, bool want_rows = false, double h = 0.0);
+  bool build_own(const HostSystem &H, int own_size, bool want_rows = false, double h = 0.0);
 };
 
 }
diff --git a/diffcloth_amd/csrc/dc_winlib.h b/diffcloth_amd/csrc/dc_winlib.h
--- a/diffcloth_amd/csrc/dc_winlib.h
+++ b/diffcloth_amd/csrc/dc_winlib.h
@@ -88,12 +88,18 @@
 template <class V, class = void> struct vert_ignores_a : std::false_type {};
 template <class V> struct vert_ignores_a<V, std::enable_if_t<V::kIgnoresInput1>> : std::true_type {};
 
+template <class TB, class = void> struct tb_has_rows : std::false_type {};
+template <class TB> struct tb_has_rows<TB, std::void_t<decltype(std::declval<const TB &>().win_rows)>> : std::true_type {};
+template <class TB> __device__ __forceinline__ bool table_rows(const TB &S) {
+  if constexpr (tb_has_rows<TB>::value) return S.win_rows != 0; else return false;
+}
+
 template <int EB, bool PRECISE>
 struct WinTriRecs { int4 r[EB]; float4 D[EB]; float4 Dl[PRECISE ? EB : 1]; };
 template <int EB, bool PRECISE>
 struct WinBendRecs { int4 r[EB]; float4 w[EB]; float4 wl[PRECISE ? EB : 1]; };
 
-template <int THREADS, bool PRECISE = false, class TB, class Stage1, class In2, class TriOp, class BendOp, class VertOp>
+template <int THREADS, bool PRECISE = false, int ROW_PLANE = 1, int ROW_SIGN = 1, class TB, class Stage1, class In2, class TriOp, class BendOp, class VertOp>
 __device__ __forceinline__ void element_windows_t(const TB &S, int w0, int w1, float *lds, Stage1 stage1,
                                                   In2 in2, TriOp tri_op, BendOp bend_op, VertOp vert_op) {
   const int tid = threadIdx.x, lane = tid & 63;
@@ -101,6 +107,9 @@
   constexpr int MB = kWinMaxBatch;
   constexpr int VPB = 6;
   constexpr bool PAIR = THREADS < 1024;
+  const bool rows = table_rows(S);
+  const float2 *rxy = ROW_PLANE == 2 ? L.a2xy : L.a1xy;
+  const float *rz = ROW_PLANE == 2 ? L.a2z : L.a1z;
   for (int w = w0; w < w1; w++) {
     const int4 d0 = S.win[2 * w], d1 = S.win[2 * w + 1];
     const int v0 = d0.x, v1 = d0.y, lo = d0.z, vs = d0.w, toff = d1.x, nt = d1.y, boff = d1.z, nb = d1.w;
@@ -125,7 +134,7 @@
     WinBendRecs<MB, PRECISE> bcur;
     const int dump = 2 * nt + nb + 1 + lane;
     constexpr bool NOA = vert_ignores_a<VertOp>::value;
-    if (!NOA || w == w0) __syncthreads();
+    if (!NOA || rows || w == w0) __syncthreads();
     constexpr int SVR = THREADS < 1024 ? 3 : 2;
     for (int j0 = tid; j0 < vs; j0 += SVR * THREADS) {
       f3 u[SVR], sv[SVR];
@@ -268,15 +277,20 @@
         sx = fmaf(c, q.x, sx); sy = fmaf(c, q.y, sy); sz = fmaf(c, z, sz);
       }
     };
-    auto gather = [&](const int4 (&e)[VPB], int s0, int np, float &sx, float &sy, float &sz) {
+    const float2 *gxy = rows ? rxy : L.erxy;
+    const float *gz = rows ? rz : L.erz;
+    const float gsign = rows ? (float) ROW_SIGN : 1.f;
+    auto gather = [&](const int4 (&e)[VPB], int s0, int np, int own, float &sx, float &sy, float &sz) {
+      f3 ai = mk(0, 0, 0);
+      if (rows) ai = ldw(rxy, rz, own);
 #pragma unroll
       for (int j = 0; j < VPB; j++) {
-        const float on = (s0 + j < np) ? 1.f : 0.f;
-        const float2 qa = L.erxy[e[j].x], qb = L.erxy[e[j].z];
-        const float za = L.erz[e[j].x], zb = L.erz[e[j].z];
+        const float on = (s0 + j < np) ? gsign : 0.f;
+        const float2 qa = gxy[e[j].x], qb = gxy[e[j].z];
+        const float za = gz[e[j].x], zb = gz[e[j].z];
         const float ca = __int_as_float(e[j].y) * on, cb = __int_as_float(e[j].w) * on;
-        sx = fmaf(ca, qa.x, sx); sy = fmaf(ca, qa.y, sy); sz = fmaf(ca, za, sz);
-        sx = fmaf(cb, qb.x, sx); sy = fmaf(cb, qb.y, sy); sz = fmaf(cb, zb, sz);
+        sx = fmaf(ca, qa.x - ai.x, sx); sy = fmaf(ca, qa.y - ai.y, sy); sz = fmaf(ca, za - ai.z, sz);
+        sx = fmaf(cb, qb.x - ai.x, sx); sy = fmaf(cb, qb.y - ai.y, sy); sz = fmaf(cb, zb - ai.z, sz);
       }
     };
     for (int i = v0 + tid; i < v1; i += (PAIR ? 2 : 1) * THREADS) {
@@ -307,8 +321,8 @@
             gather_tri(ta1, nta > 1, ax, ay, az);
             gather_tri(tb1, ntb > 1, bx, by, bz);
           }
-          gather(ea, 0, nba, ax, ay, az);
-          gather(eb, 0, nbb, bx, by, bz);
+          gather(ea, 0, nba, i - lo, ax, ay, az);
+          gather(eb, 0, nbb, (vb ? ib : i) - lo, bx, by, bz);
         }
         for (int s0 = 2; s0 < max(nta, ntb); s0++) {
           const int4 ta = rowa[min(s0, nta - 1) * 64], tb = rowb[min(s0, ntb - 1) * 64];
@@ -319,8 +333,8 @@
           int4 ea[VPB], eb[VPB];
 #pragma unroll
           for (int j = 0; j < VPB; j++) { ea[j] = frowa[min(s0 + j, nba - 1) * 64]; eb[j] = frowb[min(s0 + j, nbb - 1) * 64]; }
-          gather(ea, s0, nba, ax, ay, az);
-          gather(eb, s0, nbb, bx, by, bz);
+          gather(ea, s0, nba, i - lo, ax, ay, az);
+          gather(eb, s0, nbb, (vb ? ib : i) - lo, bx, by, bz);
         }
         if constexpr (vert_has_pre<VertOp>::value) {
           vert_op(i, mk(ax, ay, az), ldw(L.a1xy, L.a1z, i - lo), prea);
@@ -338,14 +352,14 @@
           for (int j = 0; j < VPB; j++) ea[j] = frowa[min(j, nba - 1) * 64];
           gather_tri(ta, true, ax, ay, az);
           if (nta > 1) gather_tri(ta1, true, ax, ay, az);
-          gather(ea, 0, nba, ax, ay, az);
+          gather(ea, 0, nba, i - lo, ax, ay, az);
         }
         for (int s0 = 2; s0 < nta; s0++) gather_tri(rowa[s0 * 64], true, ax, ay, az);
         for (int s0 = VPB; s0 < nba; s0 += VPB) {
           int4 ea[VPB];
 #pragma unroll
           for (int j = 0; j < VPB; j++) ea[j] = frowa[min(s0 + j, nba - 1) * 64];
-          gather(ea, s0, nba, ax, ay, az);
+          gather(ea, s0, nba, i - lo, ax, ay, az);
         }
         if constexpr (vert_has_pre<VertOp>::value) vert_op(i, mk(ax, ay, az), ldw(L.a1xy, L.a1z, i - lo), prea);
         else vert_op(i, mk(ax, ay, az), ldw(L.a1xy, L.a1z, i - lo));
@@ -355,10 +369,10 @@
   }
 }
 
-template <int THREADS, bool PRECISE = false, class Stage1, class TriOp, class BendOp, class VertOp>
+template <int THREADS, bool PRECISE = false, int ROW_PLANE = 1, int ROW_SIGN = 1, class Stage1, class TriOp, class BendOp, class VertOp>
 __device__ __forceinline__ void element_windows(const DevSystem &S, float *lds, Stage1 stage1,
                                                 const float *__restrict__ in2, TriOp tri_op, BendOp bend_op, VertOp vert_op) {
-  element_windows_t<THREADS, PRECISE>(S, 0, S.nwin, lds, stage1, In2Plain{in2, S.N}, tri_op, bend_op, vert_op);
+  element_windows_t<THREADS, PRECISE, ROW_PLANE, ROW_SIGN>(S, 0, S.nwin, lds, stage1, In2Plain{in2, S.N}, tri_op, bend_op, vert_op);
 }
 
 struct StagePlanar {
diff --git a/include/diffcloth_hip.h b/include/diffcloth_hip.h
--- a/include/diffcloth_hip.h
+++ b/include/diffcloth_hip.h
@@ -155,6 +155,7 @@
 int dc_get_self_friction_path(dc_ctx *ctx, int *out , int reset);
 int dc_get_layout(const dc_ctx *ctx, int *out6);
 int dc_get_packet_layout(const dc_ctx *ctx, int *byte_offsets);
+int dc_get_bend_rows(const dc_ctx *ctx, int *rows);
 int dc_get_deflation(const dc_ctx *ctx, int *vectors, int *probe_iterations);
 
 int dc_comm_unique_id(char *id128 );
```
